# uci-rendering/psdr-cuda

Hardware: AMD Instinct MI355X
Metric: Mpath-samples/s renderC+renderD, cbox 512x512 spp=64; grad rel-L2 vs ref (higher is better)
Workload: dtype f32; 1 GPU; cbox 512x512 spp=64/GPU PathTracer(max_depth=3): renderC + configure + renderD + enoki.forward w.r.t. diffuse albedo, through the psdr_cuda surface; triangles=12, global_spp=64, world_size=1, device=AMD Radeon Graphics, local_rank=0

## Files before the change

__graft_entry__.py:

```python
import os
import subprocess
import sys

ROOT = os.path.dirname(os.path.abspath(__file__))
PKG = os.path.join(ROOT, "psdr-cuda_amd")
for p in (PKG, os.path.join(ROOT, "oracle"), os.path.join(ROOT, "tests")):
    if p not in sys.path:
        sys.path.insert(0, p)

HIPCC_FLAGS = ["--offload-arch=gfx950", "-O3", "-std=c++17", "-fPIC", "-munsafe-fp-atomics",
               "-fno-hip-fp32-correctly-rounded-divide-sqrt", "-fgpu-flush-denormals-to-zero", "-fno-slp-vectorize",
               "-freciprocal-math", "-fapprox-func"]
VARIANTS = (0, 1, 2, 3, 4, 6, 8, 10)


def _stale(target, sources):
    return (not os.path.exists(target)) or any(os.path.getmtime(s) > os.path.getmtime(target) for s in sources)


TESTS = os.path.join(ROOT, "tests")
CSRC = os.path.join(PKG, "csrc")
HC_DIR = os.path.join(TESTS, "hostcheck")
HOST_FLAGS = ["-O2", "-std=c++17", "-pthread"]


def _product_and_harness():
    return ([os.path.join(CSRC, f) for f in sorted(os.listdir(CSRC))] + [os.path.join(ROOT, "include", "psdr_hip.h")] +
            [os.path.join(HC_DIR, f) for f in sorted(os.listdir(HC_DIR)) if f.endswith(".h")])


TEST_LIBS = {
    "hostcheck": ("hostcheck/hostcheck.cpp", "hostcheck/libhostcheck.so", _product_and_harness, HOST_FLAGS),
    "path_sedge": ("hostcheck/hostcheck_path_sedge.cpp", "hostcheck/libhostcheck_path_sedge.so", _product_and_harness, HOST_FLAGS),
    "path_guide": ("hostcheck/hostcheck_path_guide.cpp", "hostcheck/libhostcheck_path_guide.so", _product_and_harness, HOST_FLAGS),
    "collocated": ("hostcheck/hostcheck_collocated.cpp", "hostcheck/libhostcheck_collocated.so", _product_and_harness, HOST_FLAGS),
    "pointlight": ("hostcheck/hostcheck_pointlight.cpp", "hostcheck/libhostcheck_pointlight.so", _product_and_harness, HOST_FLAGS),
    "lightstage": ("hostcheck/hostcheck_lightstage.cpp", "hostcheck/libhostcheck_lightstage.so", _product_and_harness, HOST_FLAGS),
    "distantlight": ("hostcheck/hostcheck_distantlight.cpp", "hostcheck/libhostcheck_distantlight.so", _product_and_harness, HOST_FLAGS),
    "plan": ("hostcheck/hostcheck_plan.cpp", "hostcheck/libhostcheck_plan.so", _product_and_harness, HOST_FLAGS),
    "smooth": ("hostcheck/hostcheck_smooth.cpp", "hostcheck/libhostcheck_smooth.so", lambda: [os.path.join(CSRC, "psdr_smooth.h")], HOST_FLAGS),
    "poison": ("poison/poison.hip", "poison/libpoison.so", lambda: [], ["-O1"]),
}


def testlib_deps(name):
    return [os.path.join(TESTS, TEST_LIBS[name][0])] + TEST_LIBS[name][2]()


def build_testlib(name):
    so = os.path.join(TESTS, TEST_LIBS[name][1])
    if _stale(so, testlib_deps(name)):
        subprocess.check_call(["hipcc", "--offload-arch=gfx950", "-fPIC", "-shared"] + TEST_LIBS[name][3] + [os.path.join(TESTS, TEST_LIBS[name][0]), "-o", so])
    return so


def build():
    csrc = os.path.join(PKG, "csrc")
    srcs = [os.path.join(csrc, f) for f in os.listdir(csrc)] + [os.path.join(ROOT, "include", "psdr_hip.h")]
    lib = os.path.join(PKG, "lib", "libpsdr_hip.so")
    os.makedirs(os.path.dirname(lib), exist_ok=True)
    defect_job = None
    if _stale(lib, srcs):
        obj_dir = os.path.join(PKG, "lib", "obj")
        os.makedirs(obj_dir, exist_ok=True)
        jobs, objs, unit_cmds = [], [], {}
        for v in VARIANTS:
            o = os.path.join(obj_dir, "variant%d.o" % v)
            objs.append(o)
            unit_cmds[o] = ["hipcc"] + HIPCC_FLAGS + ["-DPSDR_VARIANT_FLAGS=%d" % v, "-c", os.path.join(csrc, "psdr_variant.hip"), "-o", o]
            jobs.append(subprocess.Popen(unit_cmds[o]))
            o = os.path.join(obj_dir, "path_sedge%d.o" % v)
            objs.append(o)
            unit_cmds[o] = ["hipcc"] + HIPCC_FLAGS + ["-DPSDR_VARIANT_FLAGS=%d" % v, "-c", os.path.join(csrc, "psdr_path_sedge.hip"), "-o", o]
            jobs.append(subprocess.Popen(unit_cmds[o]))
            o = os.path.join(obj_dir, "collocated%d.o" % v)
            objs.append(o)
            unit_cmds[o] = ["hipcc"] + HIPCC_FLAGS + ["-DPSDR_VARIANT_FLAGS=%d" % v, "-c", os.path.join(csrc, "psdr_collocated.hip"), "-o", o]
            jobs.append(subprocess.Popen(unit_cmds[o]))
            o = os.path.join(obj_dir, "pointlight%d.o" % v)
            objs.append(o)
            unit_cmds[o] = ["hipcc"] + HIPCC_FLAGS + ["-DPSDR_VARIANT_FLAGS=%d" % v, "-c", os.path.join(csrc, "psdr_pointlight.hip"), "-o", o]
            jobs.append(subprocess.Popen(unit_cmds[o]))
            o = os.path.join(obj_dir, "lightstage%d.o" % v)
            objs.append(o)
            unit_cmds[o] = ["hipcc"] + HIPCC_FLAGS + ["-DPSDR_VARIANT_FLAGS=%d" % v, "-c", os.path.join(csrc, "psdr_lightstage.hip"), "-o", o]
            jobs.append(subprocess.Popen(unit_cmds[o]))
        o = os.path.join(obj_dir, "logd_lean.o")
        objs.append(o)
        unit_cmds[o] = ["hipcc"] + HIPCC_FLAGS + ["-c", os.path.join(csrc, "psdr_logd_lean.hip"), "-o", o]
        jobs.append(subprocess.Popen(unit_cmds[o]))
        o = os.path.join(obj_dir, "host.o")
        objs.append(o)
        unit_cmds[o] = ["hipcc"] + HIPCC_FLAGS + ["-c", os.path.join(csrc, "psdr_hip.hip"), "-o", o]
        jobs.append(subprocess.Popen(unit_cmds[o]))
        o = os.path.join(obj_dir, "tables.o")
        objs.append(o)
        unit_cmds[o] = ["hipcc"] + HIPCC_FLAGS + ["-c", os.path.join(csrc, "psdr_tables.hip"), "-o", o]
        jobs.append(subprocess.Popen(unit_cmds[o]))
        o = os.path.join(obj_dir, "smooth.o")
        objs.append(o)
        unit_cmds[o] = ["hipcc"] + HIPCC_FLAGS + ["-c", os.path.join(csrc, "psdr_smooth.hip"), "-o", o]
        jobs.append(subprocess.Popen(unit_cmds[o]))
        defect_job = _start_defect_object(csrc, obj_dir)
        if any(j.wait() != 0 for j in jobs):
            raise RuntimeError("hipcc failed")
        sys.path.insert(0, os.path.join(ROOT, "tools"))
        import check_spill_exec
        fallbacks = (["-mllvm", "-amdgpu-opt-exec-mask-pre-ra=0"], ["-mllvm", "-amdgpu-spill-sgpr-to-vgpr=0"])
        from concurrent.futures import ThreadPoolExecutor
        with ThreadPoolExecutor(max_workers=8) as pool:
            first = dict(zip(unit_cmds, pool.map(lambda o_: check_spill_exec.check_library(o_, verbose=True, min_code_objects=1), list(unit_cmds))))
        for o, cmd in list(unit_cmds.items()):
            hits = first[o]
            for extra in fallbacks:
                if not hits:
                    break
                print("build(): %s trips the spill guard -- rebuilding it with %s" % (os.path.basename(o), " ".join(extra)))
                subprocess.check_call(cmd[:1] + cmd[1:-4] + extra + cmd[-4:])
                hits = check_spill_exec.check_library(o, verbose=True, min_code_objects=1)
            if hits:
                raise RuntimeError("%s: %d kernel(s) spill in front of an exec restore with every fallback (tools/check_spill_exec.py)" % (os.path.basename(o), len(hits)))
        subprocess.check_call(["hipcc", "--offload-arch=gfx950", "-shared", "-fPIC"] + objs + ["-o", lib])
        if len(check_spill_exec.code_objects(lib)) < len(objs):
            raise RuntimeError("the linked library holds fewer gfx code objects than translation units: the spill guard cannot see all of it")
    subprocess.check_call(["make", "-C", os.path.join(ROOT, "oracle"), "-s"])
    for name in TEST_LIBS:
        build_testlib(name)
    try:
        build_defect_lib(defect_job)
    except Exception as e:
        print("build(): tests/poison/libpsdr_hip_defect.so not built (%s) -- only tests/test_rough_rev_order_gpu.py uses it" % e)
    import psdr_cuda
    from psdr_cuda import _abi
    _abi.load_hip()
    import oracle
    oracle.load_oracle()


def _defect_object_cmd(csrc, obj_dir):
    return ["hipcc"] + HIPCC_FLAGS + ["-DPSDR_VARIANT_FLAGS=10", "-DPSDR_SINK_REG_PRIV_ROUGH=1", "-DPSDR_DPP_ALWAYS=1", "-c",
                                      os.path.join(csrc, "psdr_variant.hip"), "-o", os.path.join(obj_dir, "variant10_defect.o")]


def _start_defect_object(csrc, obj_dir):
    try:
        return subprocess.Popen(_defect_object_cmd(csrc, obj_dir), stdout=subprocess.DEVNULL, stderr=subprocess.DEVNULL)
    except Exception:
        return None


def build_defect_lib(object_job=None):
    csrc = os.path.join(PKG, "csrc")
    srcs = [os.path.join(csrc, f) for f in os.listdir(csrc)] + [os.path.join(ROOT, "include", "psdr_hip.h")]
    obj_dir = os.path.join(PKG, "lib", "obj")
    defect_lib = os.path.join(ROOT, "tests", "poison", "libpsdr_hip_defect.so")
    objs = [os.path.join(obj_dir, "%s%d.o" % (unit, v)) for v in VARIANTS for unit in ("variant", "path_sedge", "collocated", "pointlight", "lightstage")] + [os.path.join(obj_dir, "logd_lean.o"), os.path.join(obj_dir, "host.o"), os.path.join(obj_dir, "tables.o"), os.path.join(obj_dir, "smooth.o")]
    if not all(os.path.exists(o) for o in objs):
        return None
    if object_job is not None and object_job.wait() != 0:
        object_job = None
    if _stale(defect_lib, srcs + objs):
        defect_obj = os.path.join(obj_dir, "variant10_defect.o")
        if object_job is None:
            subprocess.check_call(_defect_object_cmd(csrc, obj_dir))
        subprocess.check_call(["hipcc", "--offload-arch=gfx950", "-shared", "-fPIC"] + [defect_obj if o.endswith("variant10.o") else o for o in objs] + ["-o", defect_lib])
    return defect_lib


def smoke():
    import numpy as np
    import torch
    assert torch.cuda.is_available(), "smoke() needs a GPU"
    torch.cuda.set_device(0)
    import oracle
    from helpers import GpuScene, load_scene, rel_l2, tangents_wrt
    from psdr_cuda import _abi
    sc, P = load_scene("cbox", res=32, spp=8, sppe=4, sppse=4, translate=(0, (1.0, 0.0, 0.0)))
    tb = sc.tables(0)
    g = GpuScene(tb)
    o = _abi.make_opts(integrator=_abi.INTEGRATOR_PATH, max_depth=3, spp=8)
    img = g.render_c(o)
    ref = oracle.render(tb, o)
    assert np.isfinite(img).all() and rel_l2(img, ref) < 1e-4, rel_l2(img, ref)
    o = _abi.make_opts(spp=8, sppe=4, sppse=4)
    tan = tangents_wrt(tb, P)
    img, dimg = g.render_d_fwd(o, [tan])
    rimg, rd = oracle.render(tb, o, mode=1, tangents=tan)
    assert rel_l2(img, rimg) < 1e-4 and rel_l2(dimg[0], rd) < 1e-3, (rel_l2(img, rimg), rel_l2(dimg[0], rd))
    import psdr_cuda
    from psdr_cuda.fixtures import scene_path
    s2 = psdr_cuda.Scene()
    s2.load_file(scene_path("cbox"), False)
    s2.opts.width = s2.opts.height = 32
    s2.opts.spp, s2.opts.sppe, s2.opts.sppse, s2.opts.log_level = 4, 0, 0, 0
    s2.configure()
    out = psdr_cuda.DirectIntegrator(1, 1).renderC(s2).numpy()
    assert out.shape == (32 * 32, 3) and np.isfinite(out).all() and out.mean() > 0.05
    print("smoke OK: renderC rel-L2 vs oracle %.2e" % rel_l2(img, rimg))


if __name__ == "__main__":
    build()
    if len(sys.argv) > 1 and sys.argv[1] == "smoke":
        smoke()
    if len(sys.argv) > 1 and sys.argv[1] == "defect":
        print(build_defect_lib())
```

include/psdr_hip.h:

```cpp
#ifndef PSDR_HIP_H
#define PSDR_HIP_H

#include <stdint.h>

#ifdef __cplusplus
extern "C" {
#endif

#define PSDR_TRI_STRIDE   24
#define PSDR_TRIUV_STRIDE  8
#define PSDR_SEDGE_STRIDE 16
#define PSDR_PEDGE_STRIDE  8
#define PSDR_BSDF_STRIDE  16
#define PSDR_EMITTER_F_STRIDE 8
#define PSDR_EMITTER_I_STRIDE 4
#define PSDR_CAM_WORDS    64
#define PSDR_ENV_WORDS    32

#define PSDR_TRI_FACE_NORMALS 0x40000000

#define PSDR_BSDF_DIFFUSE        0
#define PSDR_BSDF_ROUGHCONDUCTOR 1
#define PSDR_BSDF_MICROFACET     2
#define PSDR_BSDF_MICROFACET_NORMAL 3
// ... 70 lines not shown
    const int32_t *sec_edge_faces;
    const float   *prim_edge_z;
} psdr_scene_desc;

#define PSDR_FLAG_FUSED     1
#define PSDR_FLAG_WAVEFRONT 2
#define PSDR_FLAG_LITERAL_FORMS 4
#define PSDR_FLAG_KEEP_RECORDS 8
#define PSDR_FLAG_PATH_SEDGES 16
#define PSDR_PATH_SEDGES_MAX_DEPTH 8

typedef struct psdr_render_opts {
    int32_t integrator;
    int32_t bsdf_samples, light_samples;
    int32_t max_depth;
    int32_t hide_emitters;
    int32_t field;
    int32_t spp, sppe, sppse;
    int32_t spp_begin, spp_end;
    int32_t sppe_begin, sppe_end;
    int32_t sppse_begin, sppse_end;
    int32_t flags;
    uint64_t rng_offset[3];
} psdr_render_opts;

typedef struct psdr_tangents {
    const float *d_tri_info;
    const float *d_texels;
    const float *d_emitter_rad;
    const float *d_cam_to_world;
    const float *d_sec_edge;
    const float *d_prim_edge;
    const float *d_env_f;
} psdr_tangents;

typedef struct psdr_grads {
    float *g_tri_info;
    float *g_texels;
    float *g_emitter_rad;
    float *g_cam_to_world;
    float *g_sec_edge;
    float *g_prim_edge;
    float *g_env_f;
} psdr_grads;

typedef struct psdr_scene_s *psdr_scene_t;

const char *psdr_last_error(void);
const char *psdr_version(void);
int psdr_abi_struct_sizes(int32_t out[4]);

int psdr_scene_create(psdr_scene_t *out);
int psdr_scene_destroy(psdr_scene_t h);
int psdr_scene_set_option(psdr_scene_t h, const char *name, double value);

int psdr_scene_set_tables(psdr_scene_t h, const psdr_scene_desc *desc);

int psdr_bvh_build(psdr_scene_t h, void *stream);
int psdr_bvh_stats(psdr_scene_t h, int32_t out[4]);
int psdr_scene_info(psdr_scene_t h, int32_t out[8]);

int psdr_trace(psdr_scene_t h, int32_t m,
               const float *ox, const float *oy, const float *oz,
               const float *dx, const float *dy, const float *dz,
               const float *tmax,
               int32_t *out_shape, int32_t *out_tri, float *out_u, float *out_v,
               void *stream);

int psdr_render_c(psdr_scene_t h, const psdr_render_opts *opts,
                  float *out_img, void *stream);

int psdr_render_d_fwd(psdr_scene_t h, const psdr_render_opts *opts,
                      int32_t K, const psdr_tangents *tangents,
                      float *out_img, float *out_dimg, void *stream);

int psdr_render_d_rev(psdr_scene_t h, const psdr_render_opts *opts,
                      const float *adj_img, float *out_img,
                      const psdr_grads *grads, void *stream);

int psdr_guide_build(psdr_scene_t h, const psdr_render_opts *opts,
                     const int32_t reso[4], int32_t nrounds,
                     float *out_mass, void *stream);

int psdr_scene_set_path_guide(psdr_scene_t h, const int32_t reso[3], const float *cmf, const float *pmf, float sum);
int psdr_scene_set_point_light(psdr_scene_t h, const float pos[3], int32_t K, const float *d_pos, float *g_pos);
int psdr_scene_set_point_lights(psdr_scene_t h, int32_t L, const float *pos, int32_t K, const float *d_pos, float *g_pos);
int psdr_scene_set_light(psdr_scene_t h, int32_t kind, const float v[3], int32_t K, const float *d_v, float *g_v);
int psdr_scene_set_lights(psdr_scene_t h, int32_t L, const int32_t *kinds, const float *v, int32_t K, const float *d_v, float *g_v);
int psdr_path_guide_build(psdr_scene_t h, const psdr_render_opts *opts, int32_t segment,
                          const int32_t reso[4], int32_t nrounds,
                          float *out_mass, void *stream);

int psdr_cube_sample_reuse(int32_t ndim, const int32_t *reso, const float *cmf, const float *pmf, float sum,
                           int32_t n, int32_t m, float *samples, float *out_pdf, void *stream);
int psdr_sample_boundary_segment_direct(const psdr_scene_desc *desc, int32_t m, const float *sample3,
                                        const uint8_t *active, float *out_p0, float *out_edge_dir,
                                        float *out_edge2, float *out_p2, float *out_n, float *out_pdf,
                                        uint8_t *out_valid, int32_t *out_edge, float *out_s1, void *stream);

int psdr_geo_world_vertices_fwd(int32_t V, const float *v_raw, const int32_t *vmesh, const float *mats, float *v_world, void *stream);
int psdr_geo_world_vertices_rev(int32_t V, const float *v_raw, const int32_t *vmesh, const float *mats, const float *v_world, const float *a_world, float *a_raw,
                                void *stream);
int psdr_geo_world_vertices_jvp(int32_t V, const float *v_raw, const int32_t *vmesh, const float *mats, const float *v_world, const float *t_raw, const float *t_mats,
                                float *t_world, void *stream);
int psdr_geo_tri_rows_fwd(int32_t V, int32_t T, const float *v, const int32_t *faces, float *vsum, float *rows, int32_t row_stride, void *stream);
int psdr_geo_tri_rows_rev(int32_t V, int32_t T, const float *v, const int32_t *faces, const float *vsum, const float *a_rows, int32_t row_stride,
                          float *a_vsum , float *a_v, void *stream);
int psdr_geo_tri_rows_jvp(int32_t V, int32_t T, const float *v, const int32_t *faces, const float *vsum, const float *t_v, int32_t row_stride,
                          float *t_vsum , float *t_rows, void *stream);
int psdr_geo_sec_edges_fwd(int32_t E, const int32_t *edges, const float *v, const float *rows, int32_t row_stride, float *info, uint8_t *keep, void *stream);
int psdr_geo_sec_edges_rev(int32_t E, const int32_t *edges, const float *a_info, float *a_v, float *a_rows, int32_t row_stride, void *stream);
int psdr_geo_sec_edges_jvp(int32_t E, const int32_t *edges, const float *t_v, const float *t_rows, int32_t row_stride, float *t_info, void *stream);
int psdr_geo_prim_edges_fwd(int32_t E, const int32_t *edges, const uint8_t *face_normals, const float *v, const float *rows, int32_t row_stride,
                            const float *cam22, float *rows8, float *z4, uint8_t *keep, void *stream);
int psdr_geo_prim_edges_rev(int32_t E, const int32_t *edges, const float *v, const float *cam22, const float *a_rows8, float *a_v, float *a_w2s ,
                            void *stream);
int psdr_geo_prim_edges_jvp(int32_t E, const int32_t *edges, const float *v, const float *cam22, const float *t_v, const float *t_w2s , float *t_rows8,
                            void *stream);

int psdr_geo_compact_edges_fwd(int32_t E, const float *rows, int32_t S, const uint8_t *keep, int32_t w0, int32_t wn, const void *aux, int32_t aux_stride, int32_t A,
                               void *scratch, float *rows_out, void *aux_out, int32_t *pos, float *pmf, float *cmf, float *header, void *stream);
int psdr_geo_compact_edges_rev(int32_t E, int32_t S, const int32_t *pos, const float *a_rows_out, float *a_rows, void *stream);
int psdr_geo_compact_edges_jvp(int32_t E, int32_t S, const int32_t *pos, const float *t_rows, float *t_rows_out, void *stream);
int psdr_geo_emitter_tables(int32_t M, const float *rows, int32_t row_stride, const int32_t *face_offset, const int32_t *mesh_emitter, int32_t Ne, const int32_t *emitter_i,
                            const float *radiance, const float *env_weight, float *mesh_area, float *emitter_f, float *emitter_pmf, float *emitter_cmf, float *face_pmf,
                            float *face_cmf, void *stream);

typedef struct psdr_smooth_s *psdr_smooth_t;
typedef struct psdr_smooth_info_s {
    int32_t iterations;
    int32_t converged;
    int32_t form;
    int32_t launches;
    float rel_residual[3];
    int32_t one_workgroup_limit;
    int32_t one_workgroup_default;
    int32_t num_vertices;
    int32_t num_entries;
    int32_t long_rows;
} psdr_smooth_info_t;
int psdr_smooth_create(int32_t V, int32_t F, const int32_t *faces, psdr_smooth_t *out);
void psdr_smooth_destroy(psdr_smooth_t h);
int psdr_smooth_set_option(psdr_smooth_t h, const char *name, int value);
int psdr_smooth_apply(psdr_smooth_t h, float lambda, const float *x, float *u, void *stream);
int psdr_smooth_solve(psdr_smooth_t h, float lambda, const float *b, const float *x0, float *x, float tol, int32_t max_iter, void *stream);
int psdr_smooth_info(psdr_smooth_t h, psdr_smooth_info_t *out);

int psdr_scene_rev_layout(psdr_scene_t h, int32_t out[16]);

int psdr_scene_seed_info(psdr_scene_t h, int64_t out[4]);

int psdr_scene_logd_info(psdr_scene_t h, int64_t out[4]);

int psdr_get_counters(psdr_scene_t h, uint64_t out[4]);

#ifdef __cplusplus
}
#endif
#endif
```

psdr-cuda_amd/csrc/psdr_hip.hip:

```cpp
#define PSDR_WIDE_TREE 2
#include "psdr_host.h"
#include "psdr_bvh_build.h"

#include <cstdlib>
#include <cstring>
#include <rocprim/rocprim.hpp>

namespace {
__global__ __launch_bounds__(kBlock) void k_trace(LaunchCtx cx, int m, const float *__restrict__ ox, const float *__restrict__ oy,
                                                  const float *__restrict__ oz, const float *__restrict__ dx,
                                                  const float *__restrict__ dy, const float *__restrict__ dz,
                                                  const float *__restrict__ tmax, int32_t *__restrict__ out_shape,
                                                  int32_t *__restrict__ out_tri, float *__restrict__ out_u, float *__restrict__ out_v) {
    TraversalStack st; setup_lds(cx, st);
    const SceneView &sc = cx.sc;
    for (int i = blockIdx.x * kBlock + threadIdx.x; i < m; i += gridDim.x * kBlock) {
        const Hit h = closest_hit<false, -1>(sc, st, Vec3f{ox[i], oy[i], oz[i]}, Vec3f{dx[i], dy[i], dz[i]}, tmax[i]);
        out_tri[i] = h.tri;
        out_shape[i] = h.tri >= 0 ? (sc.d.tri_mesh[h.tri] & ~PSDR_TRI_FACE_NORMALS) : -1;
        out_u[i] = h.u; out_v[i] = h.v;
    }
}


// ... 589 lines not shown
        HIP_TRY(hipMemcpyAsync(host_nodes.data(), h->d_nodes, host_nodes.size() * sizeof(BvhNode), hipMemcpyDeviceToHost, s));
        HIP_TRY(hipStreamSynchronize(s));
        if (int rc = bvh4_build(h, host_nodes, std::vector<int32_t>{0}, false, s)) return rc;
    } else { h->wide = false; h->num_nodes4 = 0; h->stack_need4 = 0; }
    h->level_start.clear();
    finish_build(h, T, info.pad, area, true, true);
    return 0;
}

int bvh4_refill(psdr_scene_s *h, hipStream_t s) {
    if (h->num_nodes4 <= 0) return 0;
    hipLaunchKernelGGL(k_bvh4_fill, dim3((h->num_nodes4 + kBlock - 1) / kBlock), dim3(kBlock), 0, s, h->d_nodes4, h->d_nodes, h->d_topo4,
                       h->d_topo4 + (size_t) h->num_nodes4 * 4, h->num_nodes4);
    HIP_TRY(hipGetLastError());
    return 0;
}
int bvh4_build(psdr_scene_s *h, const std::vector<BvhNode> &nodes, const std::vector<int32_t> &roots2, bool forest, hipStream_t s) {
    h->wide = use_wide_tree(h, forest);
    if (!h->wide && !forest) { h->num_nodes4 = 0; h->stack_need4 = 0; return 0; }
    Bvh4Topology tp;
    collapse_bvh4(nodes, roots2, tp);
    h->num_nodes4 = tp.n4; h->stack_need4 = tp.stack_need;
    h->root4 = roots2.size() == 1 ? tp.roots[0] : 0;
    for (size_t k = 0; k < roots2.size() && k < (size_t) kMaxBlas; ++k) h->blas_root4[k] = tp.roots[k];
    if (tp.n4 == 0) return 0;
    if (int rc = device_grow(h->d_nodes4, h->cap_nodes4, (size_t) tp.n4, sizeof(Bvh4Node), &h->d_topo4, 8 * sizeof(int32_t))) return rc;
    HIP_TRY(hipMemcpyAsync(h->d_topo4, tp.child.data(), (size_t) tp.n4 * 4 * sizeof(int32_t), hipMemcpyHostToDevice, s));
    HIP_TRY(hipMemcpyAsync(h->d_topo4 + (size_t) tp.n4 * 4, tp.src.data(), (size_t) tp.n4 * 4 * sizeof(int32_t), hipMemcpyHostToDevice, s));
    if (int rc = bvh4_refill(h, s)) return rc;
    HIP_TRY(hipStreamSynchronize(s));
    return 0;
}

int launch_wf_trace(psdr_scene_s *h, const float4 *req, const int32_t *count, long long sub_cap, float4 *hit, hipStream_t s, bool ign) {
    TraceArgs a{};
    a.sec_edge_faces = h->desc.sec_edge_faces;
    if (ign && !a.sec_edge_faces) ign = false;
    pack_blas_boxes(h, a.blas_lo, a.blas_hi);
    a.nodes4 = h->d_nodes4; a.btris = h->d_btris; a.req = req; a.count = count; a.hit = hit; a.sub_cap = sub_cap; a.n_blas = h->n_blas;
    const TracePlan p = plan_wf_trace(h, sub_cap);
    a.n_lnodes = p.n_lnodes; a.off_stack = p.off_stack; a.stack_entries = p.stack_entries; a.ovf_stride = p.ovf_stride;
    if (p.ovf) {
        if (int rc = scratch_reserve(reinterpret_cast<void **>(&h->d_trace_ovf), &h->trace_ovf_bytes, p.ovf_bytes, s, "trace kernel's overflow stack columns")) return rc;
        a.ovf = h->d_trace_ovf;
    }
    const bool wg2 = p.wg2, ovf = p.ovf;
    const int grid = p.grid, dyn = p.dyn;
#define PSDR_LAUNCH_TRACE_I(MULTI, OVF, IGN, WPE)                                                                                                           \
    do { static bool attr_set = false;                                                                                                                      \
         if (!attr_set) { if (int rc = allow_dynamic_lds(&k_wf_trace<MULTI, OVF, IGN, WPE>, 160 * 1024 - 1024)) return rc; attr_set = true; }                     \
         hipLaunchKernelGGL(HIP_KERNEL_NAME(k_wf_trace<MULTI, OVF, IGN, WPE>), dim3(grid), dim3(kTraceBlock), dyn, s, a); } while (0)
#define PSDR_LAUNCH_TRACE(MULTI, OVF) do { if (ign) { if (wg2) PSDR_LAUNCH_TRACE_I(MULTI, OVF, true, 8); else PSDR_LAUNCH_TRACE_I(MULTI, OVF, true, 4); } else if (wg2) PSDR_LAUNCH_TRACE_I(MULTI, OVF, false, 8); else PSDR_LAUNCH_TRACE_I(MULTI, OVF, false, 4); } while (0)
    if (h->n_blas > 1) { if (ovf) PSDR_LAUNCH_TRACE(true, true); else PSDR_LAUNCH_TRACE(true, false); }
    else { if (ovf) PSDR_LAUNCH_TRACE(false, true); else PSDR_LAUNCH_TRACE(false, false); }
#undef PSDR_LAUNCH_TRACE_I
#undef PSDR_LAUNCH_TRACE
    HIP_TRY(hipGetLastError());
    return 0;
}

int probe_buffers(psdr_scene_s *h, long long slots, int rays_per_slot, ProbeBuffers &pb, hipStream_t s, int per_cu) {
    const ProbePlan pl = plan_probe_buffers(h, slots, rays_per_slot, per_cu);
    pb.sub_cap = pl.sub_cap;
    if (int rc = scratch_reserve(&h->d_probe, &h->probe_bytes, pl.total, s, "probe buffers (hit rows, masks, trace requests)")) return rc;
    char *p = reinterpret_cast<char *>(h->d_probe);
    pb.count = reinterpret_cast<int32_t *>(p); p += pl.cnt_bytes;
    pb.hit = reinterpret_cast<float4 *>(p); p += pl.hit_bytes;
    pb.mask = reinterpret_cast<uint32_t *>(p); p += pl.mask_bytes;
    pb.req = reinterpret_cast<float4 *>(p);
    HIP_TRY(hipMemsetAsync(pb.count, 0, pl.cnt_bytes, s));
    return 0;
}

#define PSDR_OPS_OF(OPS)                                                                                                              \
    switch (scene_flag_set(h)) {                                                                                                      \
        case 0: return OPS##0(); case 1: return OPS##1(); case 2: return OPS##2(); case 3: return OPS##3();                          \
        case 4: return OPS##4(); case 8: return OPS##8(); case 10: return OPS##10();                                                 \
        default: return OPS##6();                       \
    }
const VariantOps *variant_of(const psdr_scene_s *h) { PSDR_OPS_OF(variant_ops_) }
const PathSedgeOps *path_sedge_of(const psdr_scene_s *h) { PSDR_OPS_OF(path_sedge_ops_) }
const CollocatedOps *collocated_of(const psdr_scene_s *h) { PSDR_OPS_OF(collocated_ops_) }
const PointLightOps *point_light_of(const psdr_scene_s *h) { PSDR_OPS_OF(point_light_ops_) }
const LightStageOps *light_stage_of(const psdr_scene_s *h) { PSDR_OPS_OF(light_stage_ops_) }
const char *const kDistantInEnv = "a distant light cannot reach a scene inside an environment map's bounding mesh (env_emitter >= 0)";
int check_point_light(const psdr_scene_s *h, const psdr_render_opts *o) {
    if (o->integrator == PSDR_INTEGRATOR_POINT && !h->have_point) return fail("PointLightIntegrator: no light set (psdr_scene_set_point_light)");
    if (o->integrator == PSDR_INTEGRATOR_POINT_STACK && h->stack_pos.empty()) return fail("LightStageIntegrator: no lights set (psdr_scene_set_point_lights)");
    if (h->desc.env_emitter >= 0) {
        const bool distant = o->integrator == PSDR_INTEGRATOR_POINT ? h->point_kind == PSDR_LIGHT_DISTANT
                           : o->integrator == PSDR_INTEGRATOR_POINT_STACK && std::find(h->stack_kind.begin(), h->stack_kind.end(), PSDR_LIGHT_DISTANT) != h->stack_kind.end();
        if (distant) return fail(kDistantInEnv);
    }
    return 0;
}
#undef PSDR_OPS_OF
}
using namespace psdr_host;

extern "C" {

const char *psdr_last_error(void) { return g_err.c_str(); }
const char *psdr_version(void) { return "psdr-hip 0.1 gfx950"; }
int psdr_abi_struct_sizes(int32_t out[4]) {
    out[0] = (int32_t) sizeof(psdr_scene_desc); out[1] = (int32_t) sizeof(psdr_render_opts);
    out[2] = (int32_t) sizeof(psdr_tangents); out[3] = (int32_t) sizeof(psdr_grads);
    return 0;
}

int psdr_scene_create(psdr_scene_t *out) {
    if (!out) return fail("psdr_scene_create: null output");
    psdr_scene_s *h = new psdr_scene_s();
    hipError_t e = hipMalloc(&h->d_counters, sizeof(unsigned long long) * kRayCounters * kRayCounterStride);
    if (e != hipSuccess) { delete h; return fail(std::string("hipMalloc: ") + hipGetErrorString(e)); }
    int dev = 0; hipDeviceProp_t prop;
    if (hipGetDevice(&dev) == hipSuccess && hipGetDeviceProperties(&prop, dev) == hipSuccess) {
        h->num_cus = prop.multiProcessorCount;
        h->lds_limit = (int) std::min<size_t>(prop.sharedMemPerBlock, 160 * 1024);
    }
    *out = h;
    return 0;
}

int psdr_scene_set_option(psdr_scene_t h, const char *name, double value) {
    if (!h || !name) return fail("psdr_scene_set_option: null argument");
    const std::string n(name);
    const int iv = (int) value;
    if (n == "bvh_refit") h->refit_enabled = iv != 0;
    else if (n == "forest_min_inline") { h->forest_min_inline = iv; h->have_bvh = false; }
    else if (n == "scratch_plain") g_scratch_plain = iv;
    else if (n == "own_pixels") h->opt.own_pixels = iv;
    else if (n == "emitter_pretest") h->opt.emitter_pretest = iv;
    else if (n == "occ_rows") { h->opt.occ_rows = iv; h->have_bvh = false; }
    else if (n == "aa_prims") { h->aa_enabled = iv != 0; h->have_bvh = false; }
    else if (n == "tiny_scene") h->tiny_enabled = iv != 0;
    else if (n == "two_level") h->two_level_enabled = iv != 0;
    else if (n == "wf_binned") h->wf_binned = iv != 0;
    else if (n == "wf_traced") h->traced_enabled = iv != 0;
    else if (n == "bvh_build") h->bvh_device_mode = iv;
    else if (n == "sort_edges") h->sort_edges = iv != 0;
    else if (n == "blocks_per_cu") h->opt.blocks_per_cu = iv;
    else if (n == "camera_blocks") h->opt.camera_blocks = iv;
    else if (n == "tiny_variants") h->opt.tiny_variants = iv;
    else if (n == "wide") h->opt.wide = iv;
    else if (n == "lds_budget") h->opt.lds_budget = iv;
    else if (n == "sink_rep") h->opt.sink_rep = std::max(1, std::min(16, iv));
    else if (n == "sink_private") h->opt.sink_private = iv;
    else if (n == "rev_split") h->opt.rev_split = iv;
    else if (n == "tangent_live") h->opt.tangent_live = iv;
    else if (n == "wf_geo") h->opt.wf_geo = iv;
    else if (n == "logd") h->opt.logd = iv;
    else if (n == "seed_cache") h->opt.seed_cache = iv;
    else if (n == "logd_park") h->opt.logd_park = iv;
    else if (n == "seed_cache_log2") h->opt.seed_cache_log2 = std::max(0, std::min(40, iv));
    else if (n == "keep_records") h->opt.keep_records = iv;
    else if (n == "rev_sorted") h->opt.rev_sorted = iv;
    else if (n == "sedge_split") h->opt.sedge_split = iv;
    else if (n == "pt_sedge") h->opt.pt_sedge = iv & 3;
    else if (n == "pt_sedge_walk") h->opt.pt_sedge_walk = iv;
    else if (n == "probe") h->opt.probe = iv;
    else if (n == "trace_wg2") h->opt.trace_wg2 = iv;
    else if (n == "chunk_log2") h->opt.chunk_log2 = std::max(0, std::min(30, iv));
    else if (n == "bvh_maxleaf") h->opt.bvh_maxleaf = std::max(1, std::min(8, iv));
    else if (n == "bvh_tcost") h->opt.bvh_tcost = (float) value;
    else return fail("psdr_scene_set_option: unknown option '" + n + "'");
    h->kept.valid = false;
    if (n == "tiny_scene" || n == "two_level" || n == "bvh_build" || n == "wide" || n == "bvh_maxleaf" || n == "bvh_tcost" || n == "tiny_variants") h->have_bvh = false;
    return 0;
}

int psdr_scene_destroy(psdr_scene_t h) {
    if (!h) return 0;
    if (h->d_nodes) (void) hipFree(h->d_nodes);
    if (h->d_stack_lights) (void) hipFree(h->d_stack_lights);
    if (h->d_btris) (void) hipFree(h->d_btris);
    if (h->d_counters) (void) hipFree(h->d_counters);
    if (h->d_refit_area) (void) hipFree(h->d_refit_area);
    if (h->d_sort) (void) hipFree(h->d_sort);
    if (h->d_ws) (void) hipFree(h->d_ws);
    if (h->d_live) (void) hipFree(h->d_live);
    if (h->d_logd_bad) (void) hipFree(h->d_logd_bad);
    if (h->d_seed) (void) hipFree(h->d_seed);
    if (h->seed_event) (void) hipEventDestroy(h->seed_event);
    if (h->d_hot_map) (void) hipFree(h->d_hot_map);
    if (h->d_hot_tris) (void) hipFree(h->d_hot_tris);
    if (h->d_occ) (void) hipFree(h->d_occ);
    if (h->d_top) (void) hipFree(h->d_top);
    if (h->d_inline_ids) (void) hipFree(h->d_inline_ids);
    if (h->d_lbvh) (void) hipFree(h->d_lbvh);
    if (h->d_nodes4) (void) hipFree(h->d_nodes4);
    if (h->d_topo4) (void) hipFree(h->d_topo4);
    if (h->d_rev) (void) hipFree(h->d_rev);
    if (h->d_se_list) (void) hipFree(h->d_se_list);
    if (h->d_rev_deep) (void) hipFree(h->d_rev_deep);
    if (h->d_pe_rep) (void) hipFree(h->d_pe_rep);
    if (h->d_trace_ovf) (void) hipFree(h->d_trace_ovf);
    if (h->d_probe) (void) hipFree(h->d_probe);
    delete h;
    return 0;
}

int psdr_scene_set_tables(psdr_scene_t h, const psdr_scene_desc *desc) {
    if (!h || !desc) return fail("psdr_scene_set_tables: null argument");
    psdr_scene_desc d = *desc;
    if (d.num_tris <= 0 || !d.tri_info || !d.tri_mesh) return fail("Missing meshes!");
    if (!d.cam) return fail("Missing sensor!");
    if (reinterpret_cast<uintptr_t>(d.tri_info) & 15) return fail("psdr_scene_set_tables: tri_info must be 16-byte aligned");
    if (d.width <= 0 || d.height <= 0) return fail("Invalid film resolution");
    if (d.num_meshes <= 0 || !d.mesh_bsdf || !d.mesh_emitter) return fail("psdr_scene_set_tables: mesh_bsdf / mesh_emitter missing");
    if (d.num_bsdfs > 0 && (!d.bsdf_rec || !d.texels)) return fail("psdr_scene_set_tables: bsdf_rec / texels missing");
    if (d.num_emitters > 0 && (!d.emitter_f || !d.emitter_i)) return fail("psdr_scene_set_tables: emitter tables missing");
    if (d.num_emitters > 1 && (!d.emitter_cmf || !d.emitter_pmf)) return fail("psdr_scene_set_tables: emitter distribution missing");
    if (d.num_sec_edges > 0 && (!d.sec_edge || !d.sec_cmf || !d.sec_pmf)) return fail("psdr_scene_set_tables: secondary-edge tables missing");
    if (d.num_prim_edges > 0 && (!d.prim_edge || !d.prim_cmf || !d.prim_pmf)) return fail("psdr_scene_set_tables: primary-edge tables missing");
    if (d.num_prim_edges <= 0) d.prim_edge_z = nullptr;
    if (d.num_guide_cells > 0 && (!d.guide_cmf || !d.guide_pmf)) return fail("psdr_scene_set_tables: guiding tables missing");
    if (!d.env_f) d.env_emitter = -1;
    if (d.env_emitter >= 0) {
        if (d.env_emitter >= d.num_emitters || !d.env_cmf || !d.env_pmf || d.env_reso[0] <= 0 || d.env_reso[1] <= 0 || d.env_tex[1] < 2 ||
            d.env_tex[2] < 2)
            return fail("psdr_scene_set_tables: inconsistent environment-map record");
    }
    if (h->have_tables && (d.tri_info != h->desc.tri_info || d.num_tris != h->desc.num_tris)) h->have_bvh = false;
    if (h->have_tables && (d.emitter_i != h->desc.emitter_i || d.num_emitters != h->desc.num_emitters)) h->have_bvh = false;
    if (!h->have_tables || std::memcmp(&h->desc, &d, sizeof(d)) != 0) { ++h->tables_gen; h->kept.valid = false; }
    h->desc = d;
    h->has_microfacet = (d.material_mask & ((1u << PSDR_BSDF_MICROFACET) | (1u << PSDR_BSDF_MICROFACET_NORMAL) | (1u << PSDR_BSDF_MICROFACET_HEIGHT))) != 0;
    h->has_rough = d.material_mask == 0 || (d.material_mask & (1u << PSDR_BSDF_ROUGHCONDUCTOR)) != 0 || h->has_microfacet;
    h->have_tables = true;
    h->pg_cmf = h->pg_pmf = nullptr; h->pg_sum = 0.f;
    return 0;
}

int psdr_scene_set_path_guide(psdr_scene_t h, const int32_t reso[3], const float *cmf, const float *pmf, float sum) {
    if (!h) return fail("psdr_scene_set_path_guide: null argument");
    if (!cmf) { h->pg_cmf = h->pg_pmf = nullptr; h->pg_sum = 0.f; return 0; }
    if (!reso || !pmf) return fail("psdr_scene_set_path_guide: null argument");
    if (reso[0] <= 0 || reso[1] <= 0 || reso[2] <= 0 || (long long) reso[0] * reso[1] * reso[2] > 0x7fffffffLL) return fail("psdr_scene_set_path_guide: invalid resolution");
    for (int i = 0; i < 3; ++i) h->pg_reso[i] = reso[i];
    h->pg_cmf = cmf; h->pg_pmf = pmf; h->pg_sum = sum;
    return 0;
}

static hipError_t copy_on_stream(void *dst, const void *src, size_t bytes, hipMemcpyKind kind, hipStream_t s) {
    if (hipError_t e = hipMemcpyAsync(dst, src, bytes, kind, s)) return e;
    return hipStreamSynchronize(s);
}
static void update_emit_rows(psdr_scene_s *h) {
    h->emit_rows = 0;
    if (h->n_tiny > 0 && emit_rows_wanted(h))
        h->emit_rows = tiny_emitter_rows(h->tiny_meta, h->n_tiny, h->aa_cnt, emitter_triangle_mask(h->emitter_i, h->desc.num_emitters, h->desc.num_tris));
}

static void refit_done(psdr_scene_s *h) { h->refits_since_build++; h->num_refits++; h->have_bvh = true; }
static int emitters_unchanged(psdr_scene_s *h, hipStream_t s, bool &same) {
    same = (size_t) std::max(h->desc.num_emitters, 0) * PSDR_EMITTER_I_STRIDE == h->emitter_i.size();
    if (!same || h->emitter_i.empty()) return 0;
    same = h->desc.emitter_i != nullptr;
    if (!same) return 0;
    std::vector<int32_t> now(h->emitter_i.size());
    HIP_TRY(copy_on_stream(now.data(), h->desc.emitter_i, now.size() * sizeof(int32_t), hipMemcpyDeviceToHost, s));
    same = std::memcmp(now.data(), h->emitter_i.data(), now.size() * sizeof(int32_t)) == 0;
    return 0;
}
static int host_tree_refit(psdr_scene_s *h, hipStream_t s, bool &fits) {
    fits = true;
    HIP_TRY(hipMemsetAsync(h->d_refit_area, 0, sizeof(float), s));
    hipLaunchKernelGGL(k_refit_leaves, dim3((h->num_btris + kBlock - 1) / kBlock), dim3(kBlock), 0, s, h->d_btris, h->desc.tri_info, h->num_btris);
    for (int l = (int) h->level_start.size() - 2; l >= 0; --l) {
        const int first = h->level_start[l], count = h->level_start[l + 1] - first;
        hipLaunchKernelGGL(k_refit_level, dim3((count + kBlock - 1) / kBlock), dim3(kBlock), 0, s, h->d_nodes, h->d_btris, first, count, h->bvh_pad, h->d_refit_area);
    }
    HIP_TRY(hipGetLastError());
    if (int rc = bvh4_refill(h, s)) return rc;
    if (h->n_blas == 0) return 0;
    float4 top[kMaxInlineTris * 3 + 2 * kMaxBlas];
    hipLaunchKernelGGL(k_gather_top, dim3(1), dim3(64), 0, s, h->d_top, h->d_nodes, h->desc.tri_info, h->d_inline_ids, h->n_inline, h->n_blas);
    HIP_TRY(hipMemcpyAsync(top, h->d_top, sizeof(top), hipMemcpyDeviceToHost, s));
    HIP_TRY(hipStreamSynchronize(s));
    std::vector<float4> tris(top, top + 3 * (size_t) h->n_inline), prims;
    pack_tiny_prims(tris, prims);
    fits = refit_inline_fits((int) prims.size() / 3);
    if (!fits) return 0;
    h->n_tiny = tiny_plane_form(prims, h->tiny, h->tiny_meta, &h->aa_cnt, h->aa_enabled);
    update_emit_rows(h);
    for (int k = 0; k < h->n_blas; ++k) {
        const float w = h->blas_lo[k].w;
        h->blas_lo[k] = top[kMaxInlineTris * 3 + k]; h->blas_lo[k].w = w;
        h->blas_hi[k] = top[kMaxInlineTris * 3 + kMaxBlas + k];
    }
    return 0;
}
static int try_refit(psdr_scene_s *h, int T, bool tiny, hipStream_t s, bool &done) {
    done = false;
    if (!refit_candidate(h, T, tiny)) return 0;
    bool emitters_same = false;
    if (int rc = emitters_unchanged(h, s, emitters_same)) return rc;
    const bool stands = forest_stands(h);
    if (refit_choice(h, emitters_same, stands, h->built_area) == kRefitNone) return 0;
    float prev_area = h->built_area;
    if (h->refits_since_build > 0) {
        HIP_TRY(hipMemcpyAsync(&prev_area, h->d_refit_area, sizeof(float), hipMemcpyDeviceToHost, h->refit_stream));
        HIP_TRY(hipStreamSynchronize(h->refit_stream));
    }
    const RefitKind kind = refit_choice(h, emitters_same, stands, prev_area);
    if (kind == kRefitNone) return 0;
// ... 228 lines not shown
    if (pos == nullptr || L == 0) return 0;
    if (int rc = device_grow(h->d_stack_lights, h->cap_stack_lights, (size_t) L, sizeof(float) * 13)) return rc;
    h->stack_pos.assign(pos, pos + 3 * (size_t) L);
    h->stack_kind.assign((size_t) L, PSDR_LIGHT_POINT);
    if (d_pos != nullptr && K > 0) { h->stack_K = K; h->stack_dpos.assign(d_pos, d_pos + 3 * (size_t) L * K); }
    h->stack_gpos = g_pos;
    return 0;
}

static int check_light_vector(const char *fn, int kind, const float *v, const std::string &which) {
    if (kind != PSDR_LIGHT_POINT && kind != PSDR_LIGHT_DISTANT) return fail(std::string(fn) + ": unknown light kind " + std::to_string(kind) + which + " (PSDR_LIGHT_POINT or PSDR_LIGHT_DISTANT)");
    if (kind != PSDR_LIGHT_DISTANT || v == nullptr) return 0;
    if (!(std::isfinite(v[0]) && std::isfinite(v[1]) && std::isfinite(v[2]))) return fail(std::string(fn) + ": the direction" + which + " is not finite");
    if (v[0] == 0.f && v[1] == 0.f && v[2] == 0.f) return fail(std::string(fn) + ": the direction" + which + " is all zero");
    return 0;
}

int psdr_scene_set_light(psdr_scene_t h, int32_t kind, const float v[3], int32_t K, const float *d_v, float *g_v) {
    if (!h) return fail("psdr_scene_set_light: null handle");
    if (int rc = check_light_vector("psdr_scene_set_light", kind, v, "")) return rc;
    if (int rc = psdr_scene_set_point_light(h, v, K, d_v, g_v)) return rc;
    if (v != nullptr) h->point_kind = kind;
    return 0;
}

int psdr_scene_set_lights(psdr_scene_t h, int32_t L, const int32_t *kinds, const float *v, int32_t K, const float *d_v, float *g_v) {
    if (!h) return fail("psdr_scene_set_lights: null handle");
    const bool some = v != nullptr && L != 0;
    if (some && kinds == nullptr) return fail("psdr_scene_set_lights: null kinds");
    if (some && L >= 1 && L <= PSDR_POINT_LIGHTS_MAX)
        for (int l = 0; l < L; ++l)
            if (int rc = check_light_vector("psdr_scene_set_lights", kinds[l], v + 3 * l, " of light " + std::to_string(l))) return rc;
    if (int rc = psdr_scene_set_point_lights(h, L, v, K, d_v, g_v)) return rc;
    if (some) h->stack_kind.assign(kinds, kinds + L);
    return 0;
}

int psdr_guide_build(psdr_scene_t h, const psdr_render_opts *o, const int32_t reso[4], int32_t nrounds, float *out_mass, void *stream) {
    if (!h || !o || !reso || !out_mass) return fail("psdr_guide_build: null argument");
    if (int rc = check_microfacet(h, o)) return rc;
    if (nrounds <= 0) return fail("psdr_guide_build: nrounds must be positive");
    if (h->desc.num_sec_edges <= 0) return fail("psdr_guide_build: scene has no secondary edges");
    hipStream_t s = (hipStream_t) stream;
    if (int rc = begin_call(h, s)) return rc;
    LaunchCtx cx;
    if (int rc = make_ctx(h, o, 2, cx)) return rc;
    cx.sc.d.guide_cmf = nullptr; cx.sc.d.num_guide_cells = 0;
    const long long cells = (long long) reso[0] * reso[1] * reso[2];
    const long long n = cells * reso[3];
    if (n <= 0 || n > 0x7fffffffLL) return fail("psdr_guide_build: invalid resolution");
    HIP_TRY(hipMemsetAsync(out_mass, 0, sizeof(float) * cells, s));
    return variant_of(h)->guide(h, cx, reso, nrounds, n, out_mass, s);
}

int psdr_path_guide_build(psdr_scene_t h, const psdr_render_opts *o, int32_t segment, const int32_t reso[4], int32_t nrounds, float *out_mass, void *stream) {
    if (!h || !o || !reso || !out_mass) return fail("psdr_path_guide_build: null argument");
    if (int rc = check_microfacet(h, o)) return rc;
    if (nrounds <= 0) return fail("psdr_path_guide_build: nrounds must be positive");
    if (o->integrator != PSDR_INTEGRATOR_PATH) return fail("psdr_path_guide_build: the integrator must be PSDR_INTEGRATOR_PATH");
    if (o->max_depth < 1) return fail("psdr_path_guide_build: max_depth must be at least 1");
    if (o->max_depth > PSDR_PATH_SEDGES_MAX_DEPTH) return fail("psdr_path_guide_build: PathTracer max_depth > 8 is not supported for the secondary-edge term");
    if (segment != 1 && segment != 2) return fail("psdr_path_guide_build: segment must be 1 (direct source) or 2 (indirect source)");
    if (segment == 2 && o->max_depth < 2) return fail("psdr_path_guide_build: segment 2 needs max_depth >= 2");
    if (!h->have_tables) return fail("Scene not loaded yet!");
    if (h->desc.num_sec_edges <= 0) return fail("psdr_path_guide_build: scene has no secondary edges");
    if (reso[0] <= 0 || reso[1] <= 0 || reso[2] <= 0 || reso[3] <= 0) return fail("psdr_path_guide_build: invalid resolution");
    const long long cells = (long long) reso[0] * reso[1] * reso[2];
    if (cells > 0x7fffffffLL || cells * reso[3] > 0x7fffffffLL || cells * reso[3] * (long long) nrounds > 0x7fffffffLL)
        return fail("psdr_path_guide_build: more than 2^31 (stream, round) slots");
    hipStream_t s = (hipStream_t) stream;
    if (int rc = begin_call(h, s)) return rc;
    HIP_TRY(hipMemsetAsync(out_mass, 0, sizeof(float) * cells, s));
    return path_sedge_of(h)->guide(h, o, segment, reso, nrounds, out_mass, s);
}

int psdr_cube_sample_reuse(int32_t ndim, const int32_t *reso, const float *cmf, const float *pmf, float sum, int32_t n, int32_t m, float *samples,
                           float *out_pdf, void *stream) {
    if (!reso || !cmf || !pmf || !samples || !out_pdf) return fail("psdr_cube_sample_reuse: null argument");
    if (ndim != 2 && ndim != 3) return fail("psdr_cube_sample_reuse: ndim must be 2 or 3");
    long long cells = 1;
    for (int d = 0; d < ndim; ++d) {
        if (reso[d] <= 0) return fail("psdr_cube_sample_reuse: invalid resolution");
        cells *= reso[d];
    }
    if (cells != (long long) n) return fail("psdr_cube_sample_reuse: n must be the product of the resolution");
    if (m < 0) return fail("psdr_cube_sample_reuse: negative sample count");
    if (m == 0) return 0;
    const dim3 grid((unsigned) ((m + kBlock - 1) / kBlock));
    hipStream_t s = (hipStream_t) stream;
    if (ndim == 2)
        hipLaunchKernelGGL(k_cube_sample_reuse<2>, grid, dim3(kBlock), 0, s, m, cmf, pmf, sum, n, reso[0], reso[1], 1, samples, out_pdf);
    else
        hipLaunchKernelGGL(k_cube_sample_reuse<3>, grid, dim3(kBlock), 0, s, m, cmf, pmf, sum, n, reso[0], reso[1], reso[2], samples, out_pdf);
    HIP_TRY(hipGetLastError());
    return 0;
}

int psdr_sample_boundary_segment_direct(const psdr_scene_desc *desc, int32_t m, const float *sample3, const uint8_t *active, float *out_p0,
                                        float *out_edge_dir, float *out_edge2, float *out_p2, float *out_n, float *out_pdf, uint8_t *out_valid,
                                        int32_t *out_edge, float *out_s1, void *stream) {
    if (!desc || !sample3 || !out_p0 || !out_edge_dir || !out_edge2 || !out_p2 || !out_n || !out_pdf || !out_valid || !out_edge || !out_s1)
        return fail("psdr_sample_boundary_segment_direct: null argument");
    const psdr_scene_desc &d = *desc;
    if (d.num_sec_edges <= 0 || !d.sec_edge || !d.sec_cmf || !d.sec_pmf) return fail("Scene has no secondary edges");
    if (d.num_emitters <= 0 || !d.emitter_f || !d.emitter_i) return fail("No Emitter!");
    if (d.num_emitters > 1 && (!d.emitter_cmf || !d.emitter_pmf)) return fail("psdr_sample_boundary_segment_direct: emitter distribution missing");
    const bool env = d.env_f != nullptr && d.env_emitter >= 0;
    if (env && (d.env_emitter >= d.num_emitters || !d.env_cmf || !d.env_pmf || d.env_reso[0] <= 0 || d.env_reso[1] <= 0))
        return fail("psdr_sample_boundary_segment_direct: inconsistent environment-map record");
    if (d.num_emitters > (env ? 1 : 0) && (d.num_tris <= 0 || !d.tri_info || !d.face_cmf || !d.face_pmf))
        return fail("psdr_sample_boundary_segment_direct: area-light tables missing");
    if (m < 0) return fail("psdr_sample_boundary_segment_direct: negative sample count");
    if (m == 0) return 0;
    SceneView sc{};
    sc.d = d;
    if (!env) sc.d.env_emitter = -1;
    const dim3 grid((unsigned) ((m + kBlock - 1) / kBlock));
    hipStream_t s = (hipStream_t) stream;
    if (env)
        hipLaunchKernelGGL(k_boundary_segment_direct<kSceneEnv>, grid, dim3(kBlock), 0, s, sc, m, sample3, active, out_p0, out_edge_dir, out_edge2, out_p2, out_n,
                           out_pdf, out_valid, out_edge, out_s1);
    else
        hipLaunchKernelGGL(k_boundary_segment_direct<0>, grid, dim3(kBlock), 0, s, sc, m, sample3, active, out_p0, out_edge_dir, out_edge2, out_p2, out_n,
                           out_pdf, out_valid, out_edge, out_s1);
    HIP_TRY(hipGetLastError());
    return 0;
}

int psdr_bvh_stats(psdr_scene_t h, int32_t out[4]) {
    if (!h || !out) return fail("psdr_bvh_stats: null argument");
    out[0] = h->num_builds; out[1] = h->num_refits; out[2] = h->num_nodes; out[3] = h->bvh_depth;
    return 0;
}

int psdr_scene_info(psdr_scene_t h, int32_t out[8]) {
    if (!h || !out) return fail("psdr_scene_info: null argument");
    const int n_slab = (h->aa_cnt & 255) + ((h->aa_cnt >> 8) & 255) + (h->aa_cnt >> 16);
    out[0] = h->n_tiny - (h->aa_cnt != 0 ? kAaSlots - n_slab : 0); out[1] = h->n_blas; out[2] = h->n_inline; out[3] = h->num_btris; out[4] = h->lbvh ? 1 : 0;
    out[5] = n_slab; out[6] = h->have_occ ? 1 : 0; out[7] = h->have_occ ? h->occ_max_rows : 0;
    return 0;
}

int psdr_scene_rev_layout(psdr_scene_t h, int32_t out[16]) {
    if (!h || !out) return fail("psdr_scene_rev_layout: null argument");
    std::copy(std::begin(h->rev_layout), std::end(h->rev_layout), out);
    return 0;
}

int psdr_scene_logd_info(psdr_scene_t h, int64_t out[4]) {
    if (!h || !out) return fail("psdr_scene_logd_info: null argument");
    out[0] = h->logd_launches; out[1] = h->logd_lean_launches; out[2] = h->logd_lean_seeded; out[3] = (int64_t) h->logd_lean_lds + h->logd_lean_park;
    return 0;
}
int psdr_scene_seed_info(psdr_scene_t h, int64_t out[4]) {
    if (!h || !out) return fail("psdr_scene_seed_info: null argument");
    out[0] = h->seed_valid ? h->seed_key[0] * h->seed_key[3] : 0; out[1] = (int64_t) (h->seed_cap * sizeof(ulonglong2)); out[2] = h->seed_fills; out[3] = h->seed_launches;
    return 0;
}

int psdr_get_counters(psdr_scene_t h, uint64_t out[4]) {
    if (!h || !out) return fail("psdr_get_counters: null argument");
    unsigned long long all[kRayCounters * kRayCounterStride], c[1] = {0};
    HIP_TRY(hipMemcpyAsync(all, h->d_counters, sizeof(all), hipMemcpyDeviceToHost, h->last_stream));
    HIP_TRY(hipStreamSynchronize(h->last_stream));
    for (int i = 0; i < kRayCounters; ++i) c[0] += all[i * kRayCounterStride];
#ifdef PSDR_STAGE_CLOCKS
    {
        unsigned long long ph[12] = {0};
        for (int i = 0; i < kRayCounters; ++i) for (int k = 0; k < 12; ++k) ph[k] += all[i * kRayCounterStride + 1 + k];
        std::fprintf(stderr, "stage clocks:");
        for (int k = 0; k < 12; ++k) std::fprintf(stderr, " %llu", ph[k]);
        std::fprintf(stderr, "\n");
    }
#endif
    out[0] = c[0]; out[1] = h->slots[0]; out[2] = h->slots[1]; out[3] = h->slots[2];
    return 0;
}

}
```

psdr-cuda_amd/csrc/psdr_host.h:

```cpp
#pragma once
#include "psdr_device.h"
#include "psdr_reverse.h"

#include <algorithm>
#include <type_traits>
#include <cmath>
#include <cstdio>
#include <cstdlib>
#include <cstring>
#include <string>
#include <vector>

using namespace psdr;

struct LaunchCtx {
    SceneView sc;
    LiParams lp;
    RngJump jump;
    int32_t off_stack;
    int32_t off_pathrec;
    int32_t off_sink;
    int32_t off_park;
};

static_assert(offsetof(LaunchCtx, sc) == 0, "closest_hit reads SceneView::tiny through the kernel-argument segment pointer: LaunchCtx (SceneView first) must be the first kernel argument");

__device__ __forceinline__ void setup_lds(const LaunchCtx &cx, TraversalStack &st) {
#if defined(__HIP_DEVICE_COMPILE__)
    const SceneView &sc = cx.sc;
    float4 *dst = reinterpret_cast<float4 *>(psdr_dyn_lds);
    const float4 *src = sc.nodes4 != nullptr ? reinterpret_cast<const float4 *>(sc.nodes4) : reinterpret_cast<const float4 *>(sc.nodes);
    for (int i = threadIdx.x; i < sc.n_lnodes * 4; i += kBlock) dst[sc.off_lnodes / 16 + (i >> 2) * (kLdsNodeStride / 16) + (i & 3)] = src[i];
    for (int i = threadIdx.x; i < sc.n_lbtris * 3; i += kBlock) dst[sc.off_lbtris / 16 + i] = sc.btris[i];
    src = reinterpret_cast<const float4 *>(sc.d.tri_info);
    for (int i = threadIdx.x; i < sc.n_ltri * 6; i += kBlock) dst[sc.off_ltri / 16 + i] = src[i];
    {
        float *m = reinterpret_cast<float *>(psdr_dyn_lds + sc.off_lprim);
#pragma unroll 1
        for (int i = 0; i < sc.n_tiny; ++i) {
            int32_t tri; float k[6];
            const int w = threadIdx.x & 7;
            const float4 Sm = sc.tiny[i * 4 + 2];
            const float S[4] = {Sm.x, Sm.y, Sm.z, Sm.w};
            tiny_hit_row(sc.tiny_meta + i * 4, (threadIdx.x >> 3) & 1, tri, k, (sc.aa_cnt != 0 && i < kAaSlots) ? S : nullptr);
            const float val = w == 0 ? __int_as_float(tri) : (w == 1 ? k[0] : w == 2 ? k[1] : w == 3 ? k[2] : w == 4 ? k[3] : w == 5 ? k[4] : w == 6 ? k[5] : 0.f);
            if (threadIdx.x < kTinyHitWords) m[i * kTinyHitWords + threadIdx.x] = val;
        }
    }
    if (sc.lt_meshbsdf >= 0) {
        auto stage = [&](int off, const void *table, int words) {
            if (off < 0 || table == nullptr) return;
            const uint32_t *g = static_cast<const uint32_t *>(table);
            uint32_t *l = reinterpret_cast<uint32_t *>(psdr_dyn_lds + off);
#pragma unroll 1
            for (int i = threadIdx.x; i < words; i += kBlock) l[i] = g[i];
        };
        stage(sc.lt_trimesh, sc.d.tri_mesh, sc.d.num_tris);
        stage(sc.lt_meshbsdf, sc.d.mesh_bsdf, sc.d.num_meshes);
        stage(sc.lt_meshemitter, sc.d.mesh_emitter, sc.d.num_meshes);
        stage(sc.lt_bsdf, sc.d.bsdf_rec, sc.d.num_bsdfs * PSDR_BSDF_STRIDE);
        stage(sc.lt_emf, sc.d.emitter_f, sc.d.num_emitters * PSDR_EMITTER_F_STRIDE);
        stage(sc.lt_emi, sc.d.emitter_i, sc.d.num_emitters * PSDR_EMITTER_I_STRIDE);
        stage(sc.lt_ecmf, sc.d.emitter_cmf, sc.d.num_emitters);
        stage(sc.lt_epmf, sc.d.emitter_pmf, sc.d.num_emitters);
        stage(sc.lt_fcmf, sc.d.face_cmf, sc.lt_nfaces);
        stage(sc.lt_fpmf, sc.d.face_pmf, sc.lt_nfaces);
        stage(sc.lt_uv, sc.d.tri_uv, sc.d.num_tris * PSDR_TRIUV_STRIDE);
        stage(sc.lt_tex, sc.d.texels, sc.d.num_texels);
        stage(sc.lt_occ, sc.occ, sc.d.num_tris * sc.d.num_tris);
    }
    st.base = reinterpret_cast<int32_t *>(psdr_dyn_lds + cx.off_stack) + threadIdx.x;
    __syncthreads();
#else
    (void) cx; (void) st;
#endif
}
template <class TVT> __device__ __forceinline__ void setup_lds(const LaunchCtx &cx, TraversalStack &st, const TVT &tv) {
    setup_lds(cx, st);
#if defined(__HIP_DEVICE_COMPILE__)
    if constexpr (Tab<TVT::flags>::lds_small && TVT::k > 0) {
        constexpr int K = TVT::k;
        static_assert(K <= 3, "plan_lds reserves three tangent texel pools");
        if (cx.sc.lt_tex >= 0) {
            float *l = reinterpret_cast<float *>(psdr_dyn_lds + cx.sc.lt_tex);
            const int nt = cx.sc.d.num_texels;
            for (int k = 0; k < K; ++k) {
                const float *g = tv.t[k].d_texels;
                for (int i = threadIdx.x; i < nt; i += kBlock) l[(k + 1) * nt + i] = g ? g[i] : 0.f;
            }
            __syncthreads();
        }
    }
#endif
}

constexpr int kSinkCacheWords = 6144;
struct SinkLayout {
    int tex_off, tex_n;
    int rad_off, rad_n;
    int cam_off;
    int env_off, env_n;
    int hot_off, hot_rows;
    const int32_t *hot_map, *hot_tris;
    int total;
    int rep, stride;
    int priv_off, priv_rows;
    int priv_tri[2], priv_slot[2], priv_emitter;
    int priv_regs;
    int pend_off, pend_rows;
};
constexpr int kPendWords = 10;
constexpr int kPrivRowWords = 13;
constexpr int kPrivWords = 2 * kPrivRowWords + 3;

struct psdr_scene_options {
    int blocks_per_cu = 0;
    int camera_blocks = 0;
    int tiny_variants = 1;
    int wide = -1;
    int lds_budget = 0;
    int sink_rep = 4;
    int sink_private = 1;
    int rev_split = -1;
    int tangent_live = 1;
    int wf_geo = 1;
    int own_pixels = 1;
    int emitter_pretest = 1;
    int occ_rows = 1;
    int logd = 1;
    int keep_records = 1;
    int rev_sorted = 1;
    int pt_sedge = 3;
    int pt_sedge_walk = 1;
    int sedge_split = -1;
    int chunk_log2 = 0;
    int probe = 1;
    int trace_wg2 = -1;
    int seed_cache = 1;
    int seed_cache_log2 = 25;
    int logd_park = 1;
    int bvh_maxleaf = 4;
    float bvh_tcost = 2.0f;
};

struct psdr_scene_s {
    psdr_scene_options opt;
    psdr_scene_desc desc{};
    bool have_tables = false;
    bool has_rough = true;
    int num_cus = 256;
    int lds_limit = 64 * 1024;

    BvhNode *d_nodes = nullptr;
    float4 *d_btris = nullptr;
    size_t cap_nodes = 0, cap_btris = 0;
    int32_t root = 0;
    bool have_bvh = false;
    int bvh_depth = 0, num_nodes = 0, num_btris = 0;
    Bvh4Node *d_nodes4 = nullptr;
    int32_t *d_topo4 = nullptr;
    size_t cap_nodes4 = 0;
    int num_nodes4 = 0, stack_need4 = 0;
    bool wide = false;
    int32_t *d_trace_ovf = nullptr;
    size_t trace_ovf_bytes = 0;
    bool traced_enabled = true;
    int32_t root4 = 0, blas_root4[kMaxBlas] = {};
    bool refit_enabled = true;
    int tree_tris = -1, refits_since_build = 0, num_builds = 0, num_refits = 0;
    std::vector<int> level_start;
    float bvh_pad = 0.f, built_area = 0.f;
    float *d_refit_area = nullptr;

    int bvh_device_mode = -1;
    bool lbvh = false;
    int lbvh_leaves = 0;
    void *d_lbvh = nullptr;
    size_t lbvh_bytes = 0;

    bool tiny_enabled = true, aa_enabled = true;
    int n_tiny = 0, aa_cnt = 0;
    float4 tiny[kTinyRows * 4] = {};
    int32_t tiny_meta[kTinyRows * 4] = {};
    bool two_level_enabled = true, refit_ok = true, wf_binned = true;
    int n_blas = 0, n_inline = 0;
    float4 blas_lo[kMaxBlas] = {}, blas_hi[kMaxBlas] = {};
    float4 *d_top = nullptr;
    int32_t *d_inline_ids = nullptr;

    unsigned long long *d_counters = nullptr;
    hipStream_t last_stream = nullptr;
    hipStream_t refit_stream = nullptr;
    uint64_t slots[3] = {0, 0, 0};
    int last_path_depth = 0;
    int32_t rev_layout[16] = {};

    std::vector<int32_t> emitter_i;
    int32_t *d_hot_map = nullptr, *d_hot_tris = nullptr;
    uint32_t *d_occ = nullptr; size_t occ_cap = 0; bool have_occ = false; int occ_max_rows = 0;
    int hot_rows = 0;
    bool hot_identity = false;
    size_t hot_cap = 0;

    bool sort_edges = true;
    void *d_sort = nullptr;
    size_t sort_bytes = 0;

    void *d_pe_rep = nullptr;
    size_t pe_rep_bytes = 0;

    void *d_rev_deep = nullptr;
    size_t rev_deep_bytes = 0;

    void *d_se_list = nullptr;
    size_t se_list_bytes = 0;

    void *d_rev = nullptr;
    size_t rev_bytes = 0;
    void *d_logd_bad = nullptr; size_t logd_bad_bytes = 0;
    struct KeptRecords { bool valid = false; psdr_render_opts o{}; uint64_t gen = 0; long long n = 0; int kind = 0; } kept;
    uint64_t tables_gen = 0;

    void *d_seed = nullptr;
    size_t seed_cap = 0;
    long long seed_key[4] = {0, 0, 0, 0};
    bool seed_valid = false;
    hipStream_t seed_stream = nullptr;
    hipEvent_t seed_event = nullptr;
    long long seed_fills = 0, seed_launches = 0;
    long long logd_launches = 0, logd_lean_launches = 0, logd_lean_seeded = 0;
    int logd_lean_lds = 0, logd_lean_park = 0;
    void *d_ws = nullptr;
    size_t ws_bytes = 0;
    void *d_live = nullptr;
    size_t live_bytes = 0;
    void *d_probe = nullptr;
    size_t probe_bytes = 0;
    uint32_t emit_rows = 0;
    int forest_min_inline = 0;
    int32_t pg_reso[3] = {1, 1, 1};
    const float *pg_cmf = nullptr, *pg_pmf = nullptr;
    float pg_sum = 0.f;
    bool has_microfacet = false;
    bool have_point = false;
    float point_pos[3] = {0.f, 0.f, 0.f}, point_dpos[3][3] = {};
    int point_K = 0;
    float *point_gpos = nullptr;
    int point_kind = PSDR_LIGHT_POINT;
    std::vector<float> stack_pos, stack_dpos;
    int stack_K = 0;
    float *stack_gpos = nullptr;
    std::vector<int32_t> stack_kind;
    float *d_stack_lights = nullptr;
    size_t cap_stack_lights = 0;
};

constexpr int kRayCounters = 64, kRayCounterStride = 16;
constexpr int kWfSub = 64, kWfCountStride = 32;
constexpr int kTraceBlock = 1024, kTraceNodeStride = 80, kTraceStackMax = 16;

#define HIP_TRY(expr)                                                                              \
    do { hipError_t e_ = (expr); if (e_ != hipSuccess) return psdr_host::fail(std::string(#expr) + ": " + hipGetErrorString(e_)); } while (0)
namespace psdr_host {
int fail(const std::string &m);
template <class Kernel> int allow_dynamic_lds(Kernel *kernel, int bytes) {
    if (bytes > 48 * 1024) HIP_TRY(hipFuncSetAttribute(reinterpret_cast<const void *>(kernel), hipFuncAttributeMaxDynamicSharedMemorySize, bytes));
    return 0;
}
int scratch_reserve(void **buf, size_t *have, size_t need, hipStream_t s, const char *what);
long long fit_chunk(long long chunk, size_t bytes_per_slot, size_t fixed_bytes, size_t have);
inline int workspace_reserve(psdr_scene_s *h, size_t need, hipStream_t s) { return scratch_reserve(&h->d_ws, &h->ws_bytes, need, s, "wavefront workspace (path-state streams + trace requests)"); }
void fill_top(const psdr_scene_s *h, SceneView &sc);
constexpr int kMaxInlineTris = 2 * kTinyTris;
int make_ctx(psdr_scene_s *h, const psdr_render_opts *o, int sampler, LaunchCtx &cx);
int launch_wf_trace(psdr_scene_s *h, const float4 *req, const int32_t *count, long long sub_cap, float4 *hit, hipStream_t s, bool ign = false);
struct ProbeBuffers { float4 *hit; uint32_t *mask; float4 *req; int32_t *count; long long sub_cap; };
int probe_buffers(psdr_scene_s *h, long long slots, int rays_per_slot, ProbeBuffers &pb, hipStream_t s, int per_cu = 16);
inline int sink_bytes_base(const SinkLayout &L) { return (L.priv_rows > 0 && !L.priv_regs) ? (L.priv_off + kPrivWords * kBlock) * 4 : (L.rep * L.stride * 4 + 15) / 16 * 16; }
inline int sink_bytes(const SinkLayout &L) { return L.pend_rows > 0 ? (L.pend_off + L.pend_rows * kPendWords * kBlock) * 4 : sink_bytes_base(L); }
inline void sink_reserve_pending(SinkLayout &L, int rows) { L.pend_rows = 0; L.pend_off = (sink_bytes_base(L) / 4 + 3) / 4 * 4; L.pend_rows = rows; }
int check_counts(const psdr_scene_s *h, const psdr_render_opts *o);
int check_microfacet(const psdr_scene_s *h, const psdr_render_opts *o);
int begin_call(psdr_scene_s *h, hipStream_t s);
int primary_edge_order(psdr_scene_s *h, const LaunchCtx &cx, long long i0, long long n, const uint32_t **order, hipStream_t s);
constexpr int kMaxRefits = 64;
constexpr float kRefitAreaGrowth = 1.3f;
constexpr int kLbvhAutoTris = 1 << 18;

struct VariantOps {
    int (*render_c)(psdr_scene_s *h, const psdr_render_opts *o, float *img, hipStream_t s);
    int (*render_fwd)(psdr_scene_s *h, const psdr_render_opts *o, int K, const psdr_tangents *tangents, float *img, float *dimg, hipStream_t s);
    int (*render_rev)(psdr_scene_s *h, const psdr_render_opts *o, const float *adj_img, float *out_img, const psdr_grads *grads, hipStream_t s);
    int (*guide)(psdr_scene_s *h, LaunchCtx &cx, const int32_t reso[4], int nrounds, long long n, float *out_mass, hipStream_t s);
};
struct PathSedgeOps {
    int (*fwd)(psdr_scene_s *h, const psdr_render_opts *o, int K, const psdr_tangents *tangents, float *dimg, hipStream_t s);
    int (*rev)(psdr_scene_s *h, const psdr_render_opts *o, const float *adj_img, const psdr_grads *grads, hipStream_t s);
    int (*guide)(psdr_scene_s *h, const psdr_render_opts *o, int segment, const int32_t reso[4], int nrounds, float *out_mass, hipStream_t s);
};
const PathSedgeOps *path_sedge_ops_0();
const PathSedgeOps *path_sedge_ops_1();
const PathSedgeOps *path_sedge_ops_2();
const PathSedgeOps *path_sedge_ops_3();
const PathSedgeOps *path_sedge_ops_4();
const PathSedgeOps *path_sedge_ops_6();
const PathSedgeOps *path_sedge_ops_8();
const PathSedgeOps *path_sedge_ops_10();
struct CollocatedOps {
    int (*render_c)(psdr_scene_s *h, const psdr_render_opts *o, float *img, hipStream_t s);
    int (*render_fwd)(psdr_scene_s *h, const psdr_render_opts *o, int K, const psdr_tangents *tangents, float *img, float *dimg, hipStream_t s);
    int (*render_rev)(psdr_scene_s *h, const psdr_render_opts *o, const float *adj_img, float *out_img, const psdr_grads *grads, hipStream_t s);
};
const CollocatedOps *collocated_ops_0();
const CollocatedOps *collocated_ops_1();
const CollocatedOps *collocated_ops_2();
const CollocatedOps *collocated_ops_3();
const CollocatedOps *collocated_ops_4();
const CollocatedOps *collocated_ops_6();
const CollocatedOps *collocated_ops_8();
const CollocatedOps *collocated_ops_10();
struct PointLightOps {
    int (*render_c)(psdr_scene_s *h, const psdr_render_opts *o, float *img, hipStream_t s);
    int (*render_fwd)(psdr_scene_s *h, const psdr_render_opts *o, int K, const psdr_tangents *tangents, float *img, float *dimg, hipStream_t s);
    int (*render_rev)(psdr_scene_s *h, const psdr_render_opts *o, const float *adj_img, float *out_img, const psdr_grads *grads, hipStream_t s);
    int (*edges_fwd)(psdr_scene_s *h, const psdr_render_opts *o, int K, const psdr_tangents *tangents, int kind, const float *pos, const float *d_pos, float *dimg, long long plane, hipStream_t s);
    int (*edges_rev)(psdr_scene_s *h, const psdr_render_opts *o, const float *adj_img, const psdr_grads *grads, int kind, const float *pos, float *g_pos, hipStream_t s);
};
const PointLightOps *point_light_ops_0();
const PointLightOps *point_light_ops_1();
const PointLightOps *point_light_ops_2();
const PointLightOps *point_light_ops_3();
const PointLightOps *point_light_ops_4();
const PointLightOps *point_light_ops_6();
const PointLightOps *point_light_ops_8();
const PointLightOps *point_light_ops_10();
struct LightStageOps {
    int (*render_c)(psdr_scene_s *h, const psdr_render_opts *o, float *img, hipStream_t s);
    int (*render_fwd)(psdr_scene_s *h, const psdr_render_opts *o, int K, const psdr_tangents *tangents, float *img, float *dimg, const PointLightOps *point, hipStream_t s);
    int (*render_rev)(psdr_scene_s *h, const psdr_render_opts *o, const float *adj_img, float *out_img, const psdr_grads *grads, const PointLightOps *point, hipStream_t s);
};
const LightStageOps *light_stage_ops_0();
const LightStageOps *light_stage_ops_1();
const LightStageOps *light_stage_ops_2();
const LightStageOps *light_stage_ops_3();
const LightStageOps *light_stage_ops_4();
const LightStageOps *light_stage_ops_6();
const LightStageOps *light_stage_ops_8();
const LightStageOps *light_stage_ops_10();
int logd_lean_launch_8(psdr_scene_s *h, const psdr_render_opts *o, const LaunchCtx &cx, const psdr::TangentView<1, psdr::kSceneTiny> &tv, float *img, float *dimg, hipStream_t s, bool *ran);
const VariantOps *variant_ops_0();
const VariantOps *variant_ops_1();
const VariantOps *variant_ops_2();
const VariantOps *variant_ops_3();
const VariantOps *variant_ops_4();
const VariantOps *variant_ops_6();
const VariantOps *variant_ops_8();
const VariantOps *variant_ops_10();
}

#include "psdr_plan.h"
#include "psdr_tree_plan.h"
```

psdr-cuda_amd/csrc/psdr_kernels.h:

```cpp
#pragma once
#include "psdr_host.h"

namespace {
using namespace psdr_host;

__device__ __forceinline__ float wave_shfl_down(float v, int off) { return __shfl_down(v, off, 64); }

template <int CTRL, int ROW_MASK> __device__ __forceinline__ float dpp_add(float v) {
    return v + __int_as_float(__builtin_amdgcn_update_dpp(0, __float_as_int(v), CTRL, ROW_MASK, 0xf, true));
}
__device__ __forceinline__ float wave_total(float v) {
    v = dpp_add<0x111, 0xf>(v); v = dpp_add<0x112, 0xf>(v); v = dpp_add<0x114, 0xf>(v); v = dpp_add<0x118, 0xf>(v);
    v = dpp_add<0x142, 0xa>(v); v = dpp_add<0x143, 0xc>(v);
    return __int_as_float(__builtin_amdgcn_readlane(__float_as_int(v), 63));
}
#ifndef PSDR_DPP_ALWAYS
#define PSDR_DPP_ALWAYS 0
#endif
template <int N, bool DPP = (N <= 6 || PSDR_DPP_ALWAYS)> __device__ __forceinline__ bool wave_segmented_sum(int key, float (&v)[N]) {
    const int lane = threadIdx.x & 63;
    if (DPP && __ballot(key != __builtin_amdgcn_readfirstlane(key)) == 0ull) {
#pragma unroll
        for (int i = 0; i < N; ++i) v[i] = wave_total(v[i]);
        return lane == 0;
// ... 1453 lines not shown
__global__ __launch_bounds__(kBlock) void k_secondary_edge_rev(LaunchCtx cx, DeviceSink<FL> sink, long long i0, long long n, float inv_sppse,
                                                               const float *__restrict__ adj_img, unsigned long long *counters,
                                                               const uint32_t *__restrict__ list, const int *__restrict__ list_n) {
    TraversalStack st; setup_lds(cx, st);
    sink.begin(dyn_lds_floats(cx.off_sink));
    uint32_t nrays = 0;
    const bool guided = cx.sc.d.guide_cmf != nullptr && cx.sc.d.num_guide_cells > 0;
    if (list != nullptr) n = *list_n;
    for (long long jj = (long long) blockIdx.x * kBlock + threadIdx.x; jj < n; jj += (long long) gridDim.x * kBlock) {
        const long long j = list != nullptr ? (long long) list[jj] : jj;
        Rng rng; rng.init((uint64_t) (i0 + j), cx.jump);
        float s3[3] = {rng.next(), rng.next(), rng.next()};
        const float pdf0 = guided ? guide_sample_reuse(cx.sc, s3) : 1.f;
        secondary_edge_reverse(sink, cx.sc, st, s3, (pdf0 > kEpsilon ? 1.f / pdf0 : 1.f) * inv_sppse, adj_img, nrays, list == nullptr);
    }
    sink.end();
    count_rays(counters, nrays);
}


template <int FL> int make_device_sink(const psdr_scene_s *h, const psdr_grads *grads, DeviceSink<FL> &sink) {
    sink.g = *grads; sink.L = make_sink_layout(h, grads);
    if ((FL & kSceneTiny) != 0 && PSDR_TINY_DIRECT_ROWS && grads->g_tri_info != nullptr && !(h->hot_identity && sink.L.hot_rows == h->desc.num_tris))
        return fail("psdr_render_d_rev: the gradient cache of a scene without a tree does not hold every triangle row");
    return 0;
}
inline bool tangents_move_geometry(const psdr_tangents *tangents, int K) {
    bool geo = false;
    for (int k = 0; k < K; ++k) geo = geo || tangents[k].d_tri_info || tangents[k].d_cam_to_world;
    return geo;
}
struct EdgeLaunch { LaunchCtx cx; long long i0, n; const uint32_t *order; };
inline int begin_edge_term(psdr_scene_s *h, const psdr_render_opts *o, int sampler, EdgeLaunch &e, hipStream_t s) {
    if (int rc = make_ctx(h, o, sampler, e.cx)) return rc;
    const long long WH = (long long) h->desc.width * h->desc.height;
    const int begin = sampler == 1 ? o->sppe_begin : o->sppse_begin, end = sampler == 1 ? o->sppe_end : o->sppse_end;
    e.i0 = WH * begin; e.n = WH * (end - begin);
    h->slots[sampler] += (uint64_t) e.n;
    e.order = nullptr;
    return sampler == 1 ? primary_edge_order(h, e.cx, e.i0, e.n, &e.order, s) : 0;
}
template <int FL> int begin_pe_replicas(psdr_scene_s *h, const psdr_grads *grads, const EdgeLaunch &e, PrimaryEdgeSink<FL> &pe_sink, hipStream_t s) {
    const long long pe_words = (long long) h->desc.num_prim_edges * PSDR_PEDGE_STRIDE;
    const int reps = primary_edge_replicas(pe_words, e.n);
    if (reps > 1) {
        const size_t need = (size_t) reps * pe_words * sizeof(float);
        if (int rc = scratch_reserve(&h->d_pe_rep, &h->pe_rep_bytes, need, s, "primary-edge gradient replicas")) return rc;
        HIP_TRY(hipMemsetAsync(h->d_pe_rep, 0, need, s));
    }
    pe_sink = PrimaryEdgeSink<FL>{reps > 1 ? reinterpret_cast<float *>(h->d_pe_rep) : grads->g_prim_edge, pe_words, reps};
    h->rev_layout[9] = reps; h->rev_layout[15] = e.order != nullptr ? 1 : 0;
    return 0;
}
template <int FL> int end_pe_replicas(psdr_scene_s *h, const psdr_grads *grads, const PrimaryEdgeSink<FL> &pe_sink, hipStream_t s) {
    if (pe_sink.reps > 1) {
        hipLaunchKernelGGL(k_sum_replicas, dim3((unsigned) ((pe_sink.rep_stride + kBlock - 1) / kBlock)), dim3(kBlock), 0, s, grads->g_prim_edge,
                           reinterpret_cast<const float *>(h->d_pe_rep), pe_sink.rep_stride, pe_sink.reps);
        HIP_TRY(hipGetLastError());
    }
    return 0;
}
template <int FL> int probe_and_trace(psdr_scene_s *h, const psdr_render_opts *o, const LaunchCtx &cx, long long c0, long long nc, ProbeBuffers &pb, hipStream_t s) {
    const int probe_per_cu = big_launch_per_cu(h, nc);
    if (int rc = probe_buffers(h, nc, 3, pb, s, probe_per_cu)) return rc;
    const TraceQueue tq{pb.req, pb.count, pb.sub_cap};
    const int blocks = (launch_blocks(h, nc, probe_per_cu) + kWfSub - 1) / kWfSub * kWfSub;
    hipLaunchKernelGGL(k_direct_probe<FL>, dim3(blocks), dim3(kBlock), lds_bytes(cx, h), s, cx, TangentView<0, FL>{}, o->spp, o->spp_begin, SlotDiv(o->spp_end - o->spp_begin), c0, nc, tq,
                       pb.hit, pb.mask, make_rng_jump(o->rng_offset[0] + 2));
    HIP_TRY(hipGetLastError());
    return launch_wf_trace(h, pb.req, pb.count, pb.sub_cap, pb.hit, s);
}
inline const ulonglong2 *seed_table(psdr_scene_s *h, const psdr_render_opts *o, long long WH, int nsp, long long n, hipStream_t s) {
    if (h->opt.seed_cache == 0 || n <= 0 || n > (1ll << std::max(0, std::min(40, h->opt.seed_cache_log2)))) return nullptr;
    const long long key[4] = {WH, (long long) o->spp, (long long) o->spp_begin, (long long) nsp};
    if (h->d_seed != nullptr && h->seed_valid && std::equal(key, key + 4, h->seed_key)) {
        if (s != h->seed_stream && h->seed_event != nullptr && hipStreamWaitEvent(s, h->seed_event, 0) != hipSuccess) { (void) hipGetLastError(); return nullptr; }
        return reinterpret_cast<const ulonglong2 *>(h->d_seed);
    }
    h->seed_valid = false;
    if ((size_t) n > h->seed_cap) {
        if (h->d_seed) { (void) hipFreeAsync(h->d_seed, s); h->d_seed = nullptr; h->seed_cap = 0; }
        void *nb = nullptr;
        if (hipMallocAsync(&nb, (size_t) n * sizeof(ulonglong2), s) != hipSuccess) { (void) hipGetLastError(); return nullptr; }
        h->d_seed = nb; h->seed_cap = (size_t) n;
    }
    if (h->seed_event == nullptr && hipEventCreateWithFlags(&h->seed_event, hipEventDisableTiming) != hipSuccess) { (void) hipGetLastError(); h->seed_event = nullptr; return nullptr; }
    hipLaunchKernelGGL(k_seed_fill, dim3((unsigned) ((n + kBlock - 1) / kBlock)), dim3(kBlock), 0, s, reinterpret_cast<ulonglong2 *>(h->d_seed), n, o->spp, o->spp_begin, SlotDiv(nsp));
    if (hipGetLastError() != hipSuccess || hipEventRecord(h->seed_event, s) != hipSuccess) { (void) hipGetLastError(); return nullptr; }
    std::copy(key, key + 4, h->seed_key);
    h->seed_valid = true; h->seed_stream = s; h->seed_fills++;
    return reinterpret_cast<const ulonglong2 *>(h->d_seed);
}
template <class G, class R, int FL> constexpr bool seeded_render_c() { return (FL & kSceneTiny) != 0 && (FL & kScenePre) == 0 && std::is_same<G, float>::value && std::is_same<R, float>::value; }
template <class G, class R, int FL>
int run_camera(psdr_scene_s *h, const psdr_render_opts *o, const TV<R, FL> &tv, float *img, float *dimg, hipStream_t s) {
    const long long WH = (long long) h->desc.width * h->desc.height;
    const int nsp = o->spp_end - o->spp_begin;
    if (o->spp <= 0 || nsp <= 0) return 0;
    LaunchCtx cx;
    if (int rc = make_ctx(h, o, 0, cx)) return rc;
    const long long n = WH * nsp;
    h->slots[0] += (uint64_t) n;
    if constexpr ((FL & kSceneForest) != 0) {
        if (o->integrator == PSDR_INTEGRATOR_DIRECT && probe_direct(h, o, n)) {
            TV<R, FL | kScenePre> tvp;
            for (int k = 0; k < (ad_traits<R>::K > 0 ? ad_traits<R>::K : 1); ++k) tvp.t[k] = tv.t[k];
            tvp.live = tv.live;
            LaunchCtx cxp = cx;
            plan_lds_no_walk(h, cxp);
            const long long chunk = std::min<long long>(n, launch_chunk(h, 25));
            const int own = wave_owns_pixels(h, nsp, chunk);
            for (long long c0 = 0; c0 < n; c0 += chunk) {
                const long long nc = std::min(chunk, n - c0);
                ProbeBuffers pb;
                if (int rc = probe_and_trace<FL>(h, o, cx, c0, nc, pb, s)) return rc;
                hipLaunchKernelGGL(HIP_KERNEL_NAME(k_camera<G, R, PSDR_INTEGRATOR_DIRECT, FL | kScenePre, false>), dim3(launch_blocks(h, nc, camera_blocks_per_cu(h, nc))), dim3(kBlock), cxp.off_stack, s,
                                   cxp, tvp, o->spp, o->spp_begin, SlotDiv(nsp), nc, 1.f / (float) o->spp, img, dimg, WH * 3, h->d_counters, c0, ProbeView{pb.hit, pb.mask}, own);
                HIP_TRY(hipGetLastError());
            }
            return 0;
        }
    }
    const int own = wave_owns_pixels(h, nsp, n);
    bool gated = false;
    if constexpr (logd_instance<G, R, PSDR_INTEGRATOR_PATH, FL>()) {
        constexpr int K = ad_traits<R>::K;
        bool texels_only = o->integrator == PSDR_INTEGRATOR_PATH && h->opt.logd != 0 && h->desc.num_texels > 0 && h->desc.texels != nullptr;
        for (int k = 0; k < K && texels_only; ++k) {
            const psdr_tangents &t = tv.t[k];
            texels_only = t.d_texels != nullptr && !t.d_tri_info && !t.d_emitter_rad && !t.d_cam_to_world && !t.d_sec_edge && !t.d_prim_edge && !t.d_env_f;
        }
        if (texels_only) {
            if (int rc = scratch_reserve(&h->d_logd_bad, &h->logd_bad_bytes, sizeof(int), s, "log-derivative gate")) return rc;
            int *bad = reinterpret_cast<int *>(h->d_logd_bad);
            HIP_TRY(hipMemsetAsync(bad, 0, sizeof(int), s));
            TangentView<K, 0> tvk;
            for (int k = 0; k < K; ++k) tvk.t[k] = tv.t[k];
            hipLaunchKernelGGL(k_logd_check<K>, dim3((unsigned) ((h->desc.num_texels + kBlock - 1) / kBlock)), dim3(kBlock), 0, s, h->desc.texels, tvk, h->desc.num_texels, h->d_counters, bad);
            hipLaunchKernelGGL(k_logd_gate, dim3(1), dim3(64), 0, s, h->d_counters, bad);
            bool lean = false;
            if constexpr (K == 1 && FL == kSceneTiny) { if (int rc = logd_lean_launch_8(h, o, cx, tv, img, dimg, s, &lean)) return rc; }
            if (!lean)
                hipLaunchKernelGGL(HIP_KERNEL_NAME(k_camera_logd<K, FL, ((FL & kSceneTiny) != 0)>), dim3(launch_blocks(h, n, camera_blocks_per_cu(h, n))), dim3(kBlock), lds_bytes(cx, h), s, cx, tv,
                                   o->spp, o->spp_begin, SlotDiv(nsp), n, 1.f / (float) o->spp, img, dimg, WH * 3, h->d_counters, own);
            HIP_TRY(hipGetLastError());
            h->logd_launches++;
            gated = true;
        }
    }
#define PSDR_LAUNCH_CAMERA_T(INTEG, NOTREE)                                                                                        \
    hipLaunchKernelGGL(HIP_KERNEL_NAME(k_camera<G, R, INTEG, FL, NOTREE>), dim3(launch_blocks(h, n, camera_blocks_per_cu(h, n))), dim3(kBlock), lds_bytes(cx, h), s, cx, tv, o->spp, \
                       o->spp_begin, nsp, n, 1.f / (float) o->spp, img, dimg, WH * 3, h->d_counters, 0ll, ProbeView{nullptr, nullptr}, own)
#define PSDR_LAUNCH_CAMERA(INTEG) PSDR_LAUNCH_CAMERA_T(INTEG, ((FL & kSceneTiny) != 0))
    if constexpr (seeded_render_c<G, R, FL>()) {
        if (o->integrator == PSDR_INTEGRATOR_PATH) {
            if (const ulonglong2 *seed = seed_table(h, o, WH, nsp, n, s)) {
                hipLaunchKernelGGL(HIP_KERNEL_NAME(k_camera_seeded<G, R, PSDR_INTEGRATOR_PATH, FL, true>), dim3(launch_blocks(h, n, camera_blocks_per_cu(h, n))), dim3(kBlock), lds_bytes(cx, h), s, cx, tv,
                                   o->spp, o->spp_begin, SlotDiv(nsp), n, 1.f / (float) o->spp, img, dimg, WH * 3, h->d_counters, own, seed);
                HIP_TRY(hipGetLastError());
                h->seed_launches++;
                return 0;
            }
        }
    }
    switch (o->integrator) {
        case PSDR_INTEGRATOR_DIRECT: PSDR_LAUNCH_CAMERA(PSDR_INTEGRATOR_DIRECT); break;
        case PSDR_INTEGRATOR_PATH: PSDR_LAUNCH_CAMERA(PSDR_INTEGRATOR_PATH); break;
        case PSDR_INTEGRATOR_FIELD: PSDR_LAUNCH_CAMERA(PSDR_INTEGRATOR_FIELD); break;
        default: return fail("Unknown integrator");
    }
#undef PSDR_LAUNCH_CAMERA
#undef PSDR_LAUNCH_CAMERA_T
    HIP_TRY(hipGetLastError());
    if (gated) HIP_TRY(hipMemsetAsync(h->d_counters + kLogdGateWord, 0, sizeof(unsigned long long), s));
    return 0;
}


constexpr int kWfMaxDepth = 256;
struct WfRecArgs { float *disk; long long stride, c0, nc; };
template <class M, int FL>
int run_camera_wavefront(psdr_scene_s *h, const psdr_render_opts *o, const TV<M, FL> &tv, float *img, float *dimg, hipStream_t s, const WfRecArgs *rec = nullptr) {
    constexpr int K = ad_traits<M>::K;
    const long long WH = (long long) h->desc.width * h->desc.height;
    const int nsp = o->spp_end - o->spp_begin;
    if (o->spp <= 0 || nsp <= 0) return 0;
    const long long n_all = WH * nsp;
    const long long n = rec ? rec->nc : n_all;
    bool traced = false;
    if constexpr ((FL & kSceneForest) != 0) traced = traced_wavefront(h);
    const bool binned = !traced && (FL & kSceneForest) != 0 && h->n_blas > 0 && h->wf_binned;
    const int depth = o->max_depth;
    const size_t words = 8 + 6 * (1 + K) + (traced ? 8 : 0);
    const long long cap = rec ? n : std::min(n, fit_chunk(binned ? launch_chunk(h, 24) : launch_chunk(h, traced ? 26 : 25), 2 * words * 4 * 5 / 4 + (traced ? 80 : 0), 64u << 20, h->ws_bytes));
    const auto wf_per_cu = [&](long long slots) { return traced ? big_launch_per_cu(h, slots) : 16; };
    const long long max_blocks = ((long long) launch_blocks(h, cap, wf_per_cu(cap)) + kWfSub - 1) / kWfSub * kWfSub;
    const long long binned_sub_cap = (((cap + kBlock - 1) / kBlock + kWfSub) / kWfGroups + 2) * kBlock;
    const long long cap_alloc = ((binned ? binned_sub_cap * kWfSub : cap + max_blocks * kBlock) + 63) / 64 * 64;
    const size_t cnt_ints = (size_t) (kWfMaxDepth + 1) * kWfStageInts + (traced ? (size_t) (kWfMaxDepth + 1) * kWfSub * kWfCountStride : 0);
    const size_t cnt_bytes = cnt_ints * sizeof(int32_t);
    const size_t req_bytes = traced ? (size_t) 2 * cap_alloc * 2 * sizeof(float4) : 0;
    const size_t need = 2 * words * 4 * (size_t) cap_alloc + cnt_bytes + req_bytes;
    if (int rc = workspace_reserve(h, need, s)) return rc;
    int32_t *cnt = reinterpret_cast<int32_t *>(h->d_ws);
    int32_t *req_cnt = cnt + (size_t) (kWfMaxDepth + 1) * kWfStageInts;
    PathStream st[2];
    for (int i = 0; i < 2; ++i) {
        float *b = reinterpret_cast<float *>(reinterpret_cast<char *>(h->d_ws) + cnt_bytes) + (size_t) i * words * cap_alloc;
        const long long c = cap_alloc;
        st[i].cap = c;
        st[i].pixel = reinterpret_cast<int32_t *>(b); st[i].slot = reinterpret_cast<uint32_t *>(b + c); st[i].tri = reinterpret_cast<int32_t *>(b + 2 * c);
        st[i].hu = b + 3 * c; st[i].hv = b + 4 * c; st[i].dir = b + 5 * c; st[i].beta = b + 8 * c; st[i].acc = b + (8 + 3 * (1 + K)) * c;
        st[i].hit = traced ? reinterpret_cast<float4 *>(b + (8 + 6 * (1 + K)) * c) : nullptr;
        st[i].prev_t = nullptr;
        st[i].binned = binned ? 1 : 0;
    }
    TraceQueue tq{};
    tq.req = traced ? reinterpret_cast<float4 *>(reinterpret_cast<char *>(h->d_ws) + cnt_bytes + 2 * words * 4 * (size_t) cap_alloc) : nullptr;
    if (!rec) h->slots[0] += (uint64_t) n;
    const float inv_spp = 1.f / (float) o->spp;
    const long long j_first = rec ? rec->c0 : 0;
    for (long long j0 = j_first; j0 < j_first + n; j0 += cap) {
        const long long cn = std::min(cap, j_first + n - j0);
        LaunchCtx cx;
        if (int rc = make_ctx(h, o, 0, cx)) return rc;
        HIP_TRY(hipMemsetAsync(cnt, 0, (size_t) (std::min(depth, kWfMaxDepth) + 1) * kWfStageInts * sizeof(int32_t), s));
        if (traced) HIP_TRY(hipMemsetAsync(req_cnt, 0, (size_t) (std::min(depth, kWfMaxDepth) + 1) * kWfSub * kWfCountStride * sizeof(int32_t), s));
        const int blocks = (launch_blocks(h, cn, wf_per_cu(cn)) + kWfSub - 1) / kWfSub * kWfSub;
        const long long trips = (cn + (long long) blocks * kBlock - 1) / ((long long) blocks * kBlock);
        st[0].sub_cap = st[1].sub_cap = binned ? binned_sub_cap : (blocks / kWfSub) * trips * kBlock;
        st[0].count = cnt;
        if constexpr ((FL & kSceneForest) != 0) {
            if (traced) {
                tq.sub_cap = 2 * st[0].sub_cap;
                tq.count = req_cnt;
                LaunchCtx cxp = cx;
                plan_lds(h, cxp, 1 << 30);
                cxp.sc.n_lnodes = cxp.sc.n_lbtris = cxp.sc.n_ltri = 0;
                const int dyn_p = cxp.off_stack;
                WfRec wr{};
                bool recording = false;
                if constexpr (K == 0) {
                    if (rec) { recording = true; wr = WfRec{rec->disk + (j0 - rec->c0), rec->stride, o->spp, o->spp_begin, nsp, j0, 0}; }
                }
                if (recording) {
                    if constexpr (K == 0)
                        hipLaunchKernelGGL(HIP_KERNEL_NAME(k_wf_camera<M, FL, true, true>), dim3(blocks), dim3(kBlock), lds_bytes(cx, h), s, cx, tv, o->spp, o->spp_begin, nsp, j0, cn,
                                           inv_spp, img, dimg, WH * 3, st[0], 1 | (depth == 1 ? 2 : 0), h->d_counters, make_rng_jump(o->rng_offset[0] + 2), tq, wr);
                } else
                hipLaunchKernelGGL(HIP_KERNEL_NAME(k_wf_camera<M, FL, true>), dim3(blocks), dim3(kBlock), lds_bytes(cx, h), s, cx, tv, o->spp, o->spp_begin, nsp, j0, cn,
                                   inv_spp, img, dimg, WH * 3, st[0], 1 | (depth == 1 ? 2 : 0), h->d_counters, make_rng_jump(o->rng_offset[0] + 2), tq, wr);
                HIP_TRY(hipGetLastError());
                for (int k = 0; k < depth; ++k) {
                    if (int rc = launch_wf_trace(h, tq.req, tq.count, tq.sub_cap, st[k & 1].hit, s)) return rc;
                    st[(k + 1) & 1].count = cnt + (size_t) (k + 1) * kWfStageInts;
                    tq.count = req_cnt + (size_t) (k + 1) * kWfSub * kWfCountStride;
                    cxp.jump = make_rng_jump(o->rng_offset[0] + 2 + 5 * (uint64_t) k);
                    wr.stage = k;
                    if (recording) {
                        if constexpr (K == 0)
                            hipLaunchKernelGGL(HIP_KERNEL_NAME(k_wf_bounce<M, FL, true, true>), dim3(blocks), dim3(kBlock), dyn_p, s, cxp, tv, inv_spp, img, dimg, WH * 3,
                                               st[k & 1], st[(k + 1) & 1], (k + 1 < depth ? 1 : 0) | (k + 2 == depth ? 2 : 0), h->d_counters, make_rng_jump(o->rng_offset[0] + 2 + 5 * (uint64_t) (k + 1)), tq, wr);
                    } else
                    hipLaunchKernelGGL(HIP_KERNEL_NAME(k_wf_bounce<M, FL, true>), dim3(blocks), dim3(kBlock), dyn_p, s, cxp, tv, inv_spp, img, dimg, WH * 3,
                                       st[k & 1], st[(k + 1) & 1], (k + 1 < depth ? 1 : 0) | (k + 2 == depth ? 2 : 0), h->d_counters, make_rng_jump(o->rng_offset[0] + 2 + 5 * (uint64_t) (k + 1)), tq, wr);
                    HIP_TRY(hipGetLastError());
                }
                continue;
            }
        }
        if (binned) {
            hipLaunchKernelGGL(HIP_KERNEL_NAME(k_wf_camera<M, FL>), dim3(blocks), dim3(kBlock), lds_bytes(cx, h), s, cx, tv, o->spp, o->spp_begin, nsp, j0, cn,
                               inv_spp, img, dimg, WH * 3, st[0], 1 | (depth == 1 ? 2 : 0), h->d_counters, make_rng_jump(o->rng_offset[0] + 2), tq, WfRec{});
            HIP_TRY(hipGetLastError());
            for (int k = 0; k < depth; ++k) {
                st[(k + 1) & 1].count = cnt + (size_t) (k + 1) * kWfStageInts;
                cx.jump = make_rng_jump(o->rng_offset[0] + 2 + 5 * (uint64_t) k);
                hipLaunchKernelGGL(HIP_KERNEL_NAME(k_wf_bounce<M, FL>), dim3(blocks), dim3(kBlock), lds_bytes(cx, h), s, cx, tv, inv_spp, img, dimg, WH * 3,
                                   st[k & 1], st[(k + 1) & 1], (k + 1 < depth ? 1 : 0) | (k + 2 == depth ? 2 : 0), h->d_counters, make_rng_jump(o->rng_offset[0] + 2 + 5 * (uint64_t) (k + 1)), tq, WfRec{});
                HIP_TRY(hipGetLastError());
            }
            continue;
        }
        hipLaunchKernelGGL(HIP_KERNEL_NAME(k_wf_camera<M, FL>), dim3(blocks), dim3(kBlock), lds_bytes(cx, h), s, cx, tv, o->spp, o->spp_begin, nsp, j0, cn,
                           inv_spp, img, dimg, WH * 3, st[0], (depth > 1 ? 1 : 0) | (depth == 2 ? 2 : 0), h->d_counters, make_rng_jump(o->rng_offset[0] + 2 + 5), tq, WfRec{});
        HIP_TRY(hipGetLastError());
        for (int k = 1; k < depth; ++k) {
            st[k & 1].count = cnt + (size_t) k * kWfStageInts;
            cx.jump = make_rng_jump(o->rng_offset[0] + 2 + 5 * (uint64_t) k);
            hipLaunchKernelGGL(HIP_KERNEL_NAME(k_wf_bounce<M, FL>), dim3(blocks), dim3(kBlock), lds_bytes(cx, h), s, cx, tv, inv_spp, img, dimg, WH * 3,
                               st[(k - 1) & 1], st[k & 1], (k + 1 < depth ? 1 : 0) | (k + 2 == depth ? 2 : 0), h->d_counters, make_rng_jump(o->rng_offset[0] + 2 + 5 * (uint64_t) (k + 1)), tq, WfRec{});
            HIP_TRY(hipGetLastError());
        }
    }
    return 0;
}

template <int K, int FL>
int run_camera_wavefront_geo(psdr_scene_s *h, const psdr_render_opts *o, const TangentView<K, FL> &tv, float *img, float *dimg, hipStream_t s) {
    const long long WH = (long long) h->desc.width * h->desc.height;
    const int nsp = o->spp_end - o->spp_begin;
    if (o->spp <= 0 || nsp <= 0) return 0;
    const long long n = WH * nsp;
    const int depth = o->max_depth;
    const size_t words = 8 + 6 * (1 + K) + 3 * K + 8;
    const long long cap = std::min(n, fit_chunk(launch_chunk(h, 26), 2 * words * 4 * 5 / 4 + 80, 64u << 20, h->ws_bytes));
// ... 357 lines not shown
```

psdr-cuda_amd/csrc/psdr_logd_lean.hip:

```cpp
#define PSDR_WIDE_TREE 0
#define PSDR_LEAF_PAIR 0
#include "psdr_kernels.h"
#include "psdr_logd_lean.h"

namespace {

constexpr int kLeanFlags = kSceneTiny;

template <int K, int FL, bool SEEDED>
__global__ __launch_bounds__(kBlock, PSDR_LOGD_WAVES_K1) void k_camera_logd_lean(LaunchCtx cx, TV<Dual<K>, FL> tv, int spp, int s_begin, SlotDiv nsp, long long n, float inv_spp,
                                                                                  float *__restrict__ img, float *__restrict__ dimg, long long plane, unsigned long long *counters, int own,
                                                                                  const ulonglong2 *__restrict__ seed) {
    constexpr int NV = 3 * (1 + K);
    if (counters[kLogdGateWord] != 1ull) return;
    TraversalStack st; setup_lds(cx, st, tv);
    Park pk{nullptr};
#if defined(__HIP_DEVICE_COMPILE__)
    pk.base = reinterpret_cast<float *>(psdr_dyn_lds + cx.off_park) + threadIdx.x;
#endif
    uint32_t nrays = 0;
    const long long nceil = (n + kBlock - 1) / kBlock * kBlock;
    for (long long jb = (long long) blockIdx.x * kBlock; jb < nceil; jb += (long long) gridDim.x * kBlock) {
        const long long j = jb + threadIdx.x;
        const bool in = j < n;
        int pixel = 0x7fffffff, s_in = 0;
        if (in) slot_to_pixel(j, nsp, pixel, s_in);
        Rng rng;
        if constexpr (SEEDED) {
            const ulonglong2 sd = in ? seed[j] : ulonglong2{0ull, 0ull};
            rng.init_seeded(sd.x, sd.y, cx.jump);
        } else {
            rng.init((uint64_t) pixel * (uint64_t) spp + (uint64_t) (s_begin + s_in), cx.jump);
        }
        const float j0 = rng.next(), j1 = rng.next();
        const int W = cx.sc.d.width;
        const float sx = ((float) (pixel % W) + j0) / (float) W, sy = ((float) (pixel / W) + j1) / (float) cx.sc.d.height;
        const TangentView<0, FL> tv0{};
        const RayT<float> ray = primary_ray<float>(cx.sc, tv0, sx, sy);
        const Vec3<Dual<K>> r = zero_nonfinite(li_path_logd_lean<K>(cx.sc, tv, st, cx.lp, rng, ray, in, nrays, pk));
        float v[NV];
        v[0] = in ? r.x.v * inv_spp : 0.f; v[1] = in ? r.y.v * inv_spp : 0.f; v[2] = in ? r.z.v * inv_spp : 0.f;
#pragma unroll
        for (int k = 0; k < K; ++k) { v[3 + 3 * k] = in ? r.x.d[k] * inv_spp : 0.f; v[4 + 3 * k] = in ? r.y.d[k] * inv_spp : 0.f; v[5 + 3 * k] = in ? r.z.d[k] * inv_spp : 0.f; }
        const bool head = wave_segmented_sum<NV>(pixel, v);
        if (head && in) {
            float *p = img + (size_t) pixel * 3;
            if (own) {
                p[0] = v[0]; p[1] = v[1]; p[2] = v[2];
#pragma unroll
                for (int k = 0; k < K; ++k) { float *q = dimg + (size_t) k * plane + (size_t) pixel * 3; q[0] = v[3 + 3 * k]; q[1] = v[4 + 3 * k]; q[2] = v[5 + 3 * k]; }
            } else {
                if (v[0] != 0.f) atomicAdd(p, v[0]);
                if (v[1] != 0.f) atomicAdd(p + 1, v[1]);
                if (v[2] != 0.f) atomicAdd(p + 2, v[2]);
#pragma unroll
                for (int k = 0; k < K; ++k) {
                    float *q = dimg + (size_t) k * plane + (size_t) pixel * 3;
                    if (v[3 + 3 * k] != 0.f) atomicAdd(q, v[3 + 3 * k]);
                    if (v[4 + 3 * k] != 0.f) atomicAdd(q + 1, v[4 + 3 * k]);
                    if (v[5 + 3 * k] != 0.f) atomicAdd(q + 2, v[5 + 3 * k]);
                }
            }
        }
    }
    count_rays(counters, nrays);
}

}

namespace psdr_host {
int logd_lean_launch_8(psdr_scene_s *h, const psdr_render_opts *o, const LaunchCtx &cx0, const psdr::TangentView<1, psdr::kSceneTiny> &tv, float *img, float *dimg, hipStream_t s, bool *ran) {
    *ran = false;
    if (h->opt.logd_park == 0) return 0;
    constexpr int kCuLds = 160 * 1024, park = ParkLayout<1>::cols * kBlock * 4;
    const int lds = (lds_bytes(cx0, h) + 15) / 16 * 16;
    const int limit = h->opt.lds_budget > 0 ? std::min(h->opt.lds_budget, kCuLds / PSDR_LOGD_WAVES_K1) : kCuLds / PSDR_LOGD_WAVES_K1;
    if (lds + park > limit) return 0;
    LaunchCtx cx = cx0;
    cx.off_park = lds;
    const long long WH = (long long) h->desc.width * h->desc.height;
    const int nsp = o->spp_end - o->spp_begin;
    const long long n = WH * nsp;
    const int own = wave_owns_pixels(h, nsp, n);
    const dim3 grid(launch_blocks(h, n, camera_blocks_per_cu(h, n)));
    const ulonglong2 *seed = seed_table(h, o, WH, nsp, n, s);
    if (seed != nullptr)
        hipLaunchKernelGGL(HIP_KERNEL_NAME(k_camera_logd_lean<1, kLeanFlags, true>), grid, dim3(kBlock), lds + park, s, cx, tv, o->spp, o->spp_begin, SlotDiv(nsp), n, 1.f / (float) o->spp, img, dimg,
                           WH * 3, h->d_counters, own, seed);
    else
        hipLaunchKernelGGL(HIP_KERNEL_NAME(k_camera_logd_lean<1, kLeanFlags, false>), grid, dim3(kBlock), lds + park, s, cx, tv, o->spp, o->spp_begin, SlotDiv(nsp), n, 1.f / (float) o->spp, img, dimg,
                           WH * 3, h->d_counters, own, seed);
    h->logd_lean_launches++;
    if (seed != nullptr) { h->logd_lean_seeded++; h->seed_launches++; }
    h->logd_lean_lds = lds; h->logd_lean_park = park;
    *ran = true;
    return 0;
}
}
```

psdr-cuda_amd/csrc/psdr_plan.h:

```cpp
#pragma once

namespace psdr_host {
inline int launch_blocks(const psdr_scene_s *h, long long n, int per_cu = 16) {
    const int forced = h->opt.blocks_per_cu;
    const long long need = (n + kBlock - 1) / kBlock;
    const long long cap = (long long) h->num_cus * (forced ? forced : per_cu);
    return (int) std::max(1LL, std::min(need, cap));
}

constexpr int kLdsBudget = 40 * 1024;
inline bool tiny_only(const psdr_scene_s *h) { return h->n_tiny > 0 && h->n_blas == 0; }
inline int emitter_faces(const psdr_scene_s *h) {
    int n = 0;
    for (int e = 0; e < h->desc.num_emitters && (size_t) (e + 1) * PSDR_EMITTER_I_STRIDE <= h->emitter_i.size(); ++e)
        n = std::max(n, h->emitter_i[(size_t) e * PSDR_EMITTER_I_STRIDE + 3] + h->emitter_i[(size_t) e * PSDR_EMITTER_I_STRIDE + 2]);
    return n;
}
constexpr int kLdsTexels = 256, kLdsTexelTangents = 3;
inline bool small_tables_fit(const psdr_scene_s *h) {
    const psdr_scene_desc &d = h->desc;
    return d.env_emitter < 0 && d.num_meshes <= 64 && d.num_bsdfs <= 32 && d.num_emitters >= 0 && d.num_emitters <= 8 &&
           (d.num_emitters == 0 || (d.face_cmf && d.face_pmf)) && emitter_faces(h) <= 64;
}
inline bool tiny_tables_ok(const psdr_scene_s *h) {
    return h->opt.tiny_variants != 0 && tiny_only(h) && small_tables_fit(h);
}
inline int scene_flag_set(const psdr_scene_s *h) {
    return (h->desc.env_emitter >= 0 ? kSceneEnv : 0) | (h->has_rough ? kSceneRough : 0) | (h->n_blas > 0 ? kSceneForest : 0) | (tiny_tables_ok(h) ? kSceneTiny : 0);
}
inline bool forest_tables(const psdr_scene_s *h) { return PSDR_FOREST_LDS_TABLES && h->n_blas > 0; }

inline int stack_entries_of(const psdr_scene_s *h) { return tiny_only(h) ? 0 : (h->wide ? h->stack_need4 + 1 : std::min(kBvhStack, h->bvh_depth + 2)); }
inline int staged_nodes_of(const psdr_scene_s *h) { return h->wide ? h->num_nodes4 : h->num_nodes; }
inline int plan_lds(const psdr_scene_s *h, LaunchCtx &cx, int reserved = 0) {
    const int forced = h->opt.lds_budget;
    const bool lean = !h->has_rough && h->desc.env_emitter < 0;
    const int budget = forced ? forced : (lean ? 28 * 1024 : kLdsBudget);
    const int stack_bytes = stack_entries_of(h) * kBlock * 4;
    int room = std::max(0, budget - reserved - stack_bytes);
    if (tiny_only(h)) room = std::max(room, staged_nodes_of(h) * kLdsNodeStride + h->num_btris * 48 + h->desc.num_tris * 96);
    SceneView &sc = cx.sc;
    int off = 0;
    sc.n_lnodes = std::min(staged_nodes_of(h), room / kLdsNodeStride); sc.off_lnodes = off; off += sc.n_lnodes * kLdsNodeStride; room -= sc.n_lnodes * kLdsNodeStride;
    sc.n_lbtris = (sc.n_lnodes == staged_nodes_of(h)) ? std::min(h->num_btris, room / 48) : 0;
    sc.off_lbtris = off; off += sc.n_lbtris * 48; room -= sc.n_lbtris * 48;
    sc.n_ltri = (sc.n_lbtris == h->num_btris) ? std::min(h->desc.num_tris, room / 96) : 0;
    sc.off_ltri = off; off += sc.n_ltri * 96;
    sc.off_lprim = off; off += h->n_tiny * kTinyHitWords * 4;
    sc.lt_trimesh = sc.lt_meshbsdf = sc.lt_meshemitter = sc.lt_bsdf = sc.lt_emf = sc.lt_emi = sc.lt_fcmf = sc.lt_fpmf = sc.lt_uv = sc.lt_tex = sc.lt_ecmf = sc.lt_epmf = -1;
    sc.lt_nfaces = 0; sc.lt_occ = -1; sc.occ = nullptr;
    const bool all_tables = tiny_tables_ok(h);
    if (all_tables || forest_tables(h)) {
        auto take = [&](int words) { const int o = off; off += (words * 4 + 15) / 16 * 16; return o; };
        const psdr_scene_desc &d = h->desc;
        sc.lt_nfaces = emitter_faces(h);
        if (all_tables) sc.lt_trimesh = take(d.num_tris);
        sc.lt_meshbsdf = take(d.num_meshes); sc.lt_meshemitter = take(d.num_meshes);
        sc.lt_bsdf = take(std::max(d.num_bsdfs, 1) * PSDR_BSDF_STRIDE);
        sc.lt_emf = take(d.num_emitters * PSDR_EMITTER_F_STRIDE); sc.lt_emi = take(d.num_emitters * PSDR_EMITTER_I_STRIDE);
        sc.lt_fcmf = take(sc.lt_nfaces); sc.lt_fpmf = take(sc.lt_nfaces);
        if (d.num_emitters > 1 && d.emitter_cmf && d.emitter_pmf) { sc.lt_ecmf = take(d.num_emitters); sc.lt_epmf = take(d.num_emitters); }
        if (all_tables && d.tri_uv) sc.lt_uv = take(d.num_tris * PSDR_TRIUV_STRIDE);
        if (d.num_texels > 0 && d.num_texels <= kLdsTexels) sc.lt_tex = take(d.num_texels * (1 + kLdsTexelTangents));
        if (all_tables && h->have_occ && h->d_occ != nullptr) { sc.occ = h->d_occ; sc.lt_occ = take(d.num_tris * d.num_tris); }
    }
    sc.lt_end = off;
    cx.off_stack = off;
    return off + stack_bytes;
}
inline int lds_bytes(const LaunchCtx &cx, const psdr_scene_s *h) { return cx.off_stack + stack_entries_of(h) * kBlock * 4; }
inline int plan_lds_no_walk(const psdr_scene_s *h, LaunchCtx &cx) {
    const int with_stacks = plan_lds(h, cx, 1 << 30);
    cx.sc.n_lnodes = cx.sc.n_lbtris = cx.sc.n_ltri = 0;
    return with_stacks;
}

inline bool open_scene(const psdr_scene_s *h) { return !(h->n_blas > 0 || (h->n_tiny > 0 && h->n_blas == 0)); }
inline bool traced_wavefront(const psdr_scene_s *h) { return h->traced_enabled && h->n_blas > 0 && h->num_nodes4 > 0 && h->d_nodes4 != nullptr; }
inline bool use_wavefront(const psdr_scene_s *h, const psdr_render_opts *o) {
    if (o->integrator != PSDR_INTEGRATOR_PATH || o->max_depth > 250) return false;
    if (h->desc.num_tris >= (1 << 29)) return false;
    if (o->flags & PSDR_FLAG_FUSED) return false;
    if (o->flags & PSDR_FLAG_WAVEFRONT) return true;
    if (o->max_depth < 2) return false;
    if (open_scene(h)) return true;
    const long long n = (long long) h->desc.width * h->desc.height * (o->spp_end - o->spp_begin);
    if (traced_wavefront(h)) return n >= (1ll << 16);
    return h->n_blas > 0 && h->wf_binned && n >= (1ll << 25);
}

inline SinkLayout make_sink_layout(const psdr_scene_s *h, const psdr_grads *g) {
    SinkLayout L{};
    int off = 0;
    L.cam_off = off; off += 16;
    if (g->g_env_f && h->desc.env_emitter >= 0) { L.env_off = off; L.env_n = PSDR_ENV_WORDS; off += PSDR_ENV_WORDS; }
    const int nt = h->desc.num_texels, nr = h->desc.num_emitters * 3;
    if (g->g_texels && nt > 0 && nt <= 2048) { L.tex_off = off; L.tex_n = nt; off += nt; }
    if (g->g_emitter_rad && nr > 0 && nr <= 256) { L.rad_off = off; L.rad_n = nr; off += nr; }
    if (g->g_tri_info && h->hot_rows > 0) {
        const int rows = std::min(h->hot_rows, (kSinkCacheWords - off) / PSDR_TRI_STRIDE);
        if (rows > 0) { L.hot_off = off; L.hot_rows = rows; L.hot_map = h->d_hot_map; L.hot_tris = h->d_hot_tris; off += rows * PSDR_TRI_STRIDE; }
    }
    L.total = off;
    L.stride = off | 1;
    L.rep = 1;
    const int max_rep = h->opt.sink_rep;
    while (L.rep * 2 <= max_rep && L.rep * 2 * L.stride <= kSinkCacheWords) L.rep *= 2;
    const bool priv_on = h->opt.sink_private != 0;
    L.priv_tri[0] = L.priv_tri[1] = -1; L.priv_slot[0] = L.priv_slot[1] = 0; L.priv_emitter = -1;
    if (priv_on && L.hot_rows > 0 && h->desc.num_emitters > 0 && h->desc.env_emitter != 0) {
        const int32_t *ei = h->emitter_i.data();
        const int n = std::min(std::min(ei[2], 2), L.hot_rows);
        for (int r = 0; r < n; ++r) { L.priv_tri[r] = ei[1] + r; L.priv_slot[r] = h->hot_identity ? ei[1] + r : r; }
        L.priv_rows = n;
        if (n > 0) { L.priv_off = (L.rep * L.stride + 3) / 4 * 4; if (L.rad_n) L.priv_emitter = 0; }
    }
    return L;
}

inline int camera_blocks_per_cu(const psdr_scene_s *h, long long n) {
    if (h->opt.camera_blocks > 0) return h->opt.camera_blocks;
    if (h->has_rough) return 16;
    if (h->n_tiny > 0 && h->n_blas == 0) return 40;
    const long long fit = n / ((long long) kBlock * h->num_cus * 2);
    return (int) std::max(16LL, std::min(64LL, fit));
}
inline int big_launch_per_cu(const psdr_scene_s *h, long long n) { return (int) std::max(16LL, std::min(40LL, n / ((long long) kBlock * h->num_cus * 8))); }
inline long long launch_chunk(const psdr_scene_s *h, int log2_default) { return 1ll << (h->opt.chunk_log2 > 0 ? h->opt.chunk_log2 : log2_default); }
inline bool probe_direct(const psdr_scene_s *h, const psdr_render_opts *o, long long n) {
    return traced_wavefront(h) && h->opt.probe != 0 && o->bsdf_samples == 1 && o->light_samples == 1 && !(o->flags & PSDR_FLAG_FUSED) && n >= (1ll << 16);
}
inline bool wave_owns_pixels(const psdr_scene_s *h, int nsp, long long chunk) {
    return h->opt.own_pixels != 0 && nsp <= 64 && 64 % nsp == 0 && chunk % nsp == 0;
}
inline bool path_sedge_split(const psdr_scene_s *h, long long n) {
    const int split_env = h->opt.sedge_split;
    return !(split_env == 0 || (split_env < 0 && n < (1ll << 18))) && n <= 0x7fffffffLL;
}
inline long long filter_grid_slots(long long n, int divisor) { return std::max(n / divisor, 1ll << 16); }
inline int primary_edge_replicas(long long pe_words, long long n) {
    int reps = 1;
    while (reps < 64 && (long long) (reps * 2) * pe_words * 4 <= (64ll << 20)) reps *= 2;
    return n < (1ll << 18) ? 1 : reps;
}

inline bool same_camera_samples(const psdr_render_opts &a, const psdr_render_opts &b) {
    return a.integrator == b.integrator && a.max_depth == b.max_depth && a.hide_emitters == b.hide_emitters && a.spp == b.spp && a.spp_begin == b.spp_begin &&
           a.spp_end == b.spp_end && a.rng_offset[0] == b.rng_offset[0] && ((a.flags ^ b.flags) & (PSDR_FLAG_FUSED | PSDR_FLAG_WAVEFRONT)) == 0;
}
inline int rev_record_words(int depth, bool wavefront) { return kRevDiskHead + (wavefront ? kRevDiskPerVertexCf : kRevDiskPerVertex) * depth; }
inline bool rev_launch_splits(const psdr_scene_s *h, const psdr_render_opts *o, long long n) {
    const int split_env = h->opt.rev_split;
    const bool replayable = o->integrator == PSDR_INTEGRATOR_PATH || (o->integrator == PSDR_INTEGRATOR_DIRECT && o->bsdf_samples <= 1 && o->light_samples <= 1);
    const bool has_tree = h->num_nodes > 0 && (h->n_tiny == 0 || h->n_blas > 0);
    const bool worth = o->integrator == PSDR_INTEGRATOR_PATH ? o->max_depth >= 2 : h->num_nodes >= 16384;
    return replayable && split_env != 0 && (split_env == 1 || (has_tree && worth && n >= (1ll << 20)));
}
inline bool rev_wavefront_sweep(const psdr_scene_s *h, const psdr_render_opts *o) {
    return o->integrator == PSDR_INTEGRATOR_PATH && std::min(o->max_depth, kMaxRevDepthDeep) <= kMaxRevDepth && traced_wavefront(h) && use_wavefront(h, o);
}
inline bool rev_value_sweep_is_wavefront(const psdr_scene_s *h, const psdr_render_opts *o, long long n) { return rev_launch_splits(h, o, n) && rev_wavefront_sweep(h, o); }

inline void rev_layout_of_sink(psdr_scene_s *h, const SinkLayout &L, bool deep_rec) {
    int32_t *r = h->rev_layout;
    r[0] = L.tex_n; r[1] = L.rad_n; r[2] = L.env_n; r[3] = L.hot_rows; r[4] = L.rep;
    r[5] = L.priv_rows; r[6] = L.priv_regs; r[7] = L.pend_rows;
    r[10] = h->hot_identity ? 1 : 0; r[11] = deep_rec ? 1 : 0; r[12] = L.priv_slot[0]; r[13] = L.priv_slot[1]; r[14] = h->hot_rows;
}

inline int plan_rev_one_vertex(const psdr_scene_s *h, LaunchCtx &cx, SinkLayout &L, int *dyn_bytes) {
    L.priv_rows = 0; L.priv_emitter = -1; L.priv_regs = 0;
    L.pend_rows = 0; L.pend_off = 0;
    const int cache_bytes = sink_bytes(L);
    plan_lds(h, cx, cache_bytes);
    cx.off_sink = lds_bytes(cx, h);
    *dyn_bytes = cx.off_sink + cache_bytes;
    if (*dyn_bytes > h->lds_limit) return fail("psdr_render_d_rev: the launch needs " + std::to_string(*dyn_bytes) + " bytes of LDS per workgroup (traversal stacks + gradient cache), the device offers " +
                                               std::to_string(h->lds_limit));
    return 0;
}

enum RevCameraForm { kRevFused = 0, kRevSplit = 1, kRevSplitWavefront = 2, kRevKeptRecords = 3, kRevProbe = 4 };
struct RevCameraPlan {
    int form, depth, rec_bytes, cache_bytes, dyn1, dyn_bytes;
    bool geo, deep_rec, split, kept_fused, no_tree;
};
inline int plan_rev_camera(psdr_scene_s *h, const psdr_render_opts *o, const psdr_grads *grads, long long n, int fl, bool reg_priv, bool value_only, bool has_out_img,
                           SinkLayout &L, LaunchCtx &cx, LaunchCtx &cx2, RevCameraPlan &p) {
    p.depth = o->integrator == PSDR_INTEGRATOR_PATH ? std::min(o->max_depth, kMaxRevDepthDeep) : 1;
    p.deep_rec = p.depth > kMaxRevDepth;
    p.rec_bytes = p.deep_rec ? 0 : p.depth * kPathRecWords * kBlock * 4;
    p.geo = value_only || grads->g_tri_info != nullptr || grads->g_cam_to_world != nullptr;
    const int wg_per_cu = (o->integrator == PSDR_INTEGRATOR_DIRECT && !(fl & kSceneRough)) ? 3 : 2;
    p.kept_fused = !value_only && p.geo && o->integrator == PSDR_INTEGRATOR_PATH && !p.deep_rec && h->opt.rev_split != 0 && h->kept.valid && h->kept.kind == 0 &&
                   h->kept.gen == h->tables_gen && h->kept.n == n && !has_out_img && same_camera_samples(h->kept.o, *o) && n <= launch_chunk(h, 26);
    p.split = value_only || p.kept_fused || (p.geo && rev_launch_splits(h, o, n));
    L.priv_regs = (p.geo && o->integrator == PSDR_INTEGRATOR_PATH && reg_priv) ? 1 : 0;
    cx2 = cx;
    const int stacks_only = plan_lds_no_walk(h, cx2);
    const int base2 = cx2.off_stack;
    const int floor_bytes = (p.split ? base2 : stacks_only) + p.rec_bytes;
    if (!L.priv_regs && L.priv_rows > 0 && floor_bytes + sink_bytes(L) > h->lds_limit / wg_per_cu) { L.priv_rows = 0; L.priv_emitter = -1; }
    L.pend_rows = 0; L.pend_off = 0;
    if (p.geo && h->opt.rev_sorted != 0 && grads->g_tri_info != nullptr && o->integrator == PSDR_INTEGRATOR_PATH) {
        for (int rows = std::min(p.depth, 4); rows >= 1; --rows) {
            SinkLayout t = L;
            sink_reserve_pending(t, rows);
            if (floor_bytes + sink_bytes(t) <= h->lds_limit / wg_per_cu) { L = t; break; }
        }
    }
    p.cache_bytes = sink_bytes(L);
    rev_layout_of_sink(h, L, p.deep_rec);
    plan_lds(h, cx, p.split ? p.rec_bytes : p.rec_bytes + p.cache_bytes);
    cx.off_pathrec = lds_bytes(cx, h);
    cx.off_sink = cx.off_pathrec + p.rec_bytes;
    cx2.off_pathrec = base2; cx2.off_sink = base2 + p.rec_bytes;
    p.no_tree = lds_bytes(cx, h) == cx.off_stack;
    if (p.split && p.no_tree) cx2 = cx;
    p.dyn1 = cx.off_pathrec + p.rec_bytes;
    p.dyn_bytes = (p.split ? cx2.off_sink : cx.off_sink) + p.cache_bytes;
    if (std::max(p.dyn_bytes, p.split ? p.dyn1 : 0) > h->lds_limit) return fail("psdr_render_d_rev: the launch needs " + std::to_string(p.dyn_bytes) + " bytes of LDS per workgroup (path record of " +
                                              std::to_string(p.depth) + " levels + traversal stacks + gradient cache), the device offers " + std::to_string(h->lds_limit));
    const bool forest = (fl & kSceneForest) != 0;
    const bool wf_value = forest && p.split && !value_only && !p.kept_fused && !p.no_tree && rev_wavefront_sweep(h, o);
    const bool direct_probe = forest && !p.split && !p.no_tree && o->integrator == PSDR_INTEGRATOR_DIRECT && probe_direct(h, o, n);
    p.form = p.split ? (wf_value ? kRevSplitWavefront : kRevSplit) : direct_probe ? kRevProbe : kRevFused;
    if (direct_probe) p.dyn_bytes = cx2.off_sink + p.cache_bytes;
    h->rev_layout[8] = p.form;
    return 0;
}
}
```

psdr-cuda_amd/psdr_cuda/_abi.py:

```python
import ctypes as C
import os

_HERE = os.path.dirname(os.path.abspath(__file__))
PKG_ROOT = os.path.dirname(_HERE)
REPO_ROOT = os.path.dirname(PKG_ROOT)

TRI_STRIDE = 24
TRIUV_STRIDE = 8
SEDGE_STRIDE = 16
PEDGE_STRIDE = 8
BSDF_STRIDE = 16
EMITTER_F_STRIDE = 8
EMITTER_I_STRIDE = 4
CAM_WORDS = 64
ENV_WORDS = 32
TRI_FACE_NORMALS = 0x40000000

BSDF_DIFFUSE, BSDF_ROUGHCONDUCTOR, BSDF_MICROFACET, BSDF_MICROFACET_NORMAL, BSDF_MICROFACET_HEIGHT = 0, 1, 2, 3, 4
SLOT_REFLECTANCE, SLOT_ALPHA_U, SLOT_ALPHA_V, SLOT_ETA, SLOT_K = range(5)
CAM_SAMPLE_TO_CAMERA, CAM_TO_WORLD, CAM_WORLD_TO_SAMPLE, CAM_POS, CAM_DIR, CAM_INV_AREA = 0, 16, 32, 48, 51, 54
INTEGRATOR_DIRECT, INTEGRATOR_PATH, INTEGRATOR_FIELD, INTEGRATOR_COLLOCATED, INTEGRATOR_POINT, INTEGRATOR_POINT_STACK = 0, 1, 2, 3, 4, 5
POINT_LIGHTS_MAX = 256
LIGHT_POINT, LIGHT_DISTANT = 0, 1
DISTANT_IN_ENV = "a distant light cannot reach a scene inside an environment map's bounding mesh (env_emitter >= 0)"
FLAG_FUSED, FLAG_WAVEFRONT, FLAG_LITERAL_FORMS, FLAG_KEEP_RECORDS, FLAG_PATH_SEDGES = 1, 2, 4, 8, 16
MAX_PATH_SEDGE_DEPTH = 8
FIELDS = {"silhouette": 0, "position": 1, "depth": 2, "geoNormal": 3, "shNormal": 4, "uv": 5}

_fp = C.c_void_p


class SceneDesc(C.Structure):
    _fields_ = [
        ("width", C.c_int32), ("height", C.c_int32),
        ("num_tris", C.c_int32), ("num_meshes", C.c_int32), ("num_bsdfs", C.c_int32), ("num_emitters", C.c_int32),
        ("num_sec_edges", C.c_int32), ("num_prim_edges", C.c_int32), ("num_texels", C.c_int32),
        ("num_guide_cells", C.c_int32),
        ("tri_info", _fp), ("tri_uv", _fp), ("tri_mesh", _fp), ("mesh_bsdf", _fp), ("mesh_emitter", _fp),
        ("bsdf_rec", _fp), ("texels", _fp), ("emitter_f", _fp), ("emitter_i", _fp),
        ("face_cmf", _fp), ("face_pmf", _fp), ("emitter_cmf", _fp), ("emitter_pmf", _fp),
        ("emitter_sum", C.c_float),
        ("cam", _fp),
        ("sec_edge", _fp), ("sec_cmf", _fp), ("sec_pmf", _fp), ("sec_sum", C.c_float),
        ("prim_edge", _fp), ("prim_cmf", _fp), ("prim_pmf", _fp), ("prim_sum", C.c_float),
        ("guide_reso", C.c_int32 * 3),
        ("guide_cmf", _fp), ("guide_pmf", _fp), ("guide_sum", C.c_float),
        ("env_emitter", C.c_int32), ("env_tex", C.c_int32 * 3), ("env_reso", C.c_int32 * 2),
        ("env_f", _fp), ("env_cmf", _fp), ("env_pmf", _fp), ("env_sum", C.c_float),
        ("material_mask", C.c_uint32),
        ("sec_edge_faces", _fp),
        ("prim_edge_z", _fp),
    ]


class RenderOpts(C.Structure):
    _fields_ = [
        ("integrator", C.c_int32), ("bsdf_samples", C.c_int32), ("light_samples", C.c_int32),
        ("max_depth", C.c_int32), ("hide_emitters", C.c_int32), ("field", C.c_int32),
        ("spp", C.c_int32), ("sppe", C.c_int32), ("sppse", C.c_int32),
        ("spp_begin", C.c_int32), ("spp_end", C.c_int32),
        ("sppe_begin", C.c_int32), ("sppe_end", C.c_int32),
        ("sppse_begin", C.c_int32), ("sppse_end", C.c_int32),
        ("flags", C.c_int32),
        ("rng_offset", C.c_uint64 * 3),
    ]


class Tangents(C.Structure):
    _fields_ = [("d_tri_info", _fp), ("d_texels", _fp), ("d_emitter_rad", _fp), ("d_cam_to_world", _fp),
                ("d_sec_edge", _fp), ("d_prim_edge", _fp), ("d_env_f", _fp)]


class Grads(C.Structure):
    _fields_ = [("g_tri_info", _fp), ("g_texels", _fp), ("g_emitter_rad", _fp), ("g_cam_to_world", _fp),
                ("g_sec_edge", _fp), ("g_prim_edge", _fp), ("g_env_f", _fp)]


class SmoothInfo(C.Structure):
    _fields_ = [("iterations", C.c_int32), ("converged", C.c_int32), ("form", C.c_int32), ("launches", C.c_int32), ("rel_residual", C.c_float * 3),
                ("one_workgroup_limit", C.c_int32), ("one_workgroup_default", C.c_int32), ("num_vertices", C.c_int32), ("num_entries", C.c_int32),
                ("long_rows", C.c_int32)]


SMOOTH_FORMS = {-1: "none", 0: "multi_launch", 1: "one_workgroup"}

TANGENT_FIELDS = ("tri_info", "texels", "emitter_rad", "cam_to_world", "sec_edge", "prim_edge", "env_f")

HIP_SYMBOLS = (
    "psdr_last_error", "psdr_version", "psdr_abi_struct_sizes", "psdr_scene_create", "psdr_scene_destroy", "psdr_scene_set_option", "psdr_scene_set_tables",
    "psdr_bvh_build", "psdr_bvh_stats", "psdr_scene_info", "psdr_trace", "psdr_render_c", "psdr_render_d_fwd", "psdr_render_d_rev",
    "psdr_guide_build", "psdr_scene_set_point_light", "psdr_scene_set_point_lights", "psdr_scene_set_light", "psdr_scene_set_lights", "psdr_scene_set_path_guide", "psdr_path_guide_build", "psdr_get_counters", "psdr_scene_rev_layout", "psdr_scene_seed_info", "psdr_scene_logd_info",
    "psdr_geo_world_vertices_fwd", "psdr_geo_world_vertices_rev", "psdr_geo_tri_rows_fwd", "psdr_geo_tri_rows_rev", "psdr_geo_sec_edges_fwd", "psdr_geo_sec_edges_rev", "psdr_geo_prim_edges_fwd", "psdr_geo_prim_edges_rev",
    "psdr_geo_compact_edges_fwd", "psdr_geo_compact_edges_rev", "psdr_geo_emitter_tables",
    "psdr_geo_world_vertices_jvp", "psdr_geo_tri_rows_jvp", "psdr_geo_sec_edges_jvp", "psdr_geo_prim_edges_jvp", "psdr_geo_compact_edges_jvp",
    "psdr_cube_sample_reuse", "psdr_sample_boundary_segment_direct",
    "psdr_smooth_create", "psdr_smooth_destroy", "psdr_smooth_set_option", "psdr_smooth_apply", "psdr_smooth_solve", "psdr_smooth_info",
)

HIP_LIB_PATH = os.path.join(PKG_ROOT, "lib", "libpsdr_hip.so")


def use_library(path):
    global HIP_LIB_PATH
    if _hip is not None:
        raise RuntimeError("psdr_cuda._abi.use_library: the library is already loaded (%s)" % HIP_LIB_PATH)
    HIP_LIB_PATH = os.path.abspath(path)


_hip = None


def load_hip():
    global _hip
    if _hip is not None:
        return _hip
    if not os.path.exists(HIP_LIB_PATH):
        raise RuntimeError("libpsdr_hip.so not built (%s): run `python -c 'import __graft_entry__ as g; g.build()'`"
                           % HIP_LIB_PATH)
    lib = C.CDLL(HIP_LIB_PATH)
    lib.psdr_last_error.restype = C.c_char_p
    lib.psdr_version.restype = C.c_char_p
    vp, i32 = C.c_void_p, C.c_int32
    lib.psdr_scene_create.argtypes = [C.POINTER(vp)]
    lib.psdr_scene_destroy.argtypes = [vp]
    lib.psdr_scene_set_option.argtypes = [vp, C.c_char_p, C.c_double]
    lib.psdr_scene_set_tables.argtypes = [vp, C.POINTER(SceneDesc)]
    lib.psdr_bvh_build.argtypes = [vp, vp]
    lib.psdr_trace.argtypes = [vp, i32] + [vp] * 7 + [vp] * 4 + [vp]
    lib.psdr_render_c.argtypes = [vp, C.POINTER(RenderOpts), vp, vp]
    lib.psdr_render_d_fwd.argtypes = [vp, C.POINTER(RenderOpts), i32, C.POINTER(Tangents), vp, vp, vp]
    lib.psdr_render_d_rev.argtypes = [vp, C.POINTER(RenderOpts), vp, vp, C.POINTER(Grads), vp]
    lib.psdr_guide_build.argtypes = [vp, C.POINTER(RenderOpts), C.POINTER(i32), i32, vp, vp]
    lib.psdr_scene_set_point_light.argtypes = [vp, C.POINTER(C.c_float), i32, C.POINTER(C.c_float), vp]
    lib.psdr_scene_set_point_lights.argtypes = [vp, i32, C.POINTER(C.c_float), i32, C.POINTER(C.c_float), vp]
    lib.psdr_scene_set_light.argtypes = [vp, i32, C.POINTER(C.c_float), i32, C.POINTER(C.c_float), vp]
    lib.psdr_scene_set_lights.argtypes = [vp, i32, C.POINTER(C.c_int32), C.POINTER(C.c_float), i32, C.POINTER(C.c_float), vp]
    lib.psdr_scene_set_path_guide.argtypes = [vp, C.POINTER(i32), vp, vp, C.c_float]
    lib.psdr_path_guide_build.argtypes = [vp, C.POINTER(RenderOpts), i32, C.POINTER(i32), i32, vp, vp]
    lib.psdr_get_counters.argtypes = [vp, C.POINTER(C.c_uint64)]
    lib.psdr_scene_info.argtypes = [vp, C.POINTER(i32)]
    lib.psdr_scene_rev_layout.argtypes = [vp, C.POINTER(i32)]
    lib.psdr_scene_seed_info.argtypes = [vp, C.POINTER(C.c_int64)]
    lib.psdr_scene_logd_info.argtypes = [vp, C.POINTER(C.c_int64)]
    lib.psdr_geo_world_vertices_fwd.argtypes = [i32, vp, vp, vp, vp, vp]
    lib.psdr_geo_world_vertices_rev.argtypes = [i32, vp, vp, vp, vp, vp, vp, vp]
    lib.psdr_geo_tri_rows_fwd.argtypes = [i32, i32, vp, vp, vp, vp, i32, vp]
    lib.psdr_geo_tri_rows_rev.argtypes = [i32, i32, vp, vp, vp, vp, i32, vp, vp, vp]
    lib.psdr_geo_sec_edges_fwd.argtypes = [i32, vp, vp, vp, i32, vp, vp, vp]
    lib.psdr_geo_sec_edges_rev.argtypes = [i32, vp, vp, vp, vp, i32, vp]
    lib.psdr_geo_prim_edges_fwd.argtypes = [i32, vp, vp, vp, vp, i32, vp, vp, vp, vp, vp]
    lib.psdr_geo_prim_edges_rev.argtypes = [i32, vp, vp, vp, vp, vp, vp, vp]
    lib.psdr_geo_compact_edges_fwd.argtypes = [i32, vp, i32, vp, i32, i32, vp, i32, i32, vp, vp, vp, vp, vp, vp, vp, vp]
    lib.psdr_geo_compact_edges_rev.argtypes = [i32, i32, vp, vp, vp, vp]
    lib.psdr_geo_world_vertices_jvp.argtypes = [i32, vp, vp, vp, vp, vp, vp, vp, vp]
    lib.psdr_geo_tri_rows_jvp.argtypes = [i32, i32, vp, vp, vp, vp, i32, vp, vp, vp]
    lib.psdr_geo_sec_edges_jvp.argtypes = [i32, vp, vp, vp, i32, vp, vp]
    lib.psdr_geo_prim_edges_jvp.argtypes = [i32, vp, vp, vp, vp, vp, vp, vp]
    lib.psdr_geo_compact_edges_jvp.argtypes = [i32, i32, vp, vp, vp, vp]
    lib.psdr_geo_emitter_tables.argtypes = [i32, vp, i32, vp, vp, i32, vp, vp, vp, vp, vp, vp, vp, vp, vp, vp]
    lib.psdr_cube_sample_reuse.argtypes = [i32, C.POINTER(i32), vp, vp, C.c_float, i32, i32, vp, vp, vp]
    lib.psdr_sample_boundary_segment_direct.argtypes = [C.POINTER(SceneDesc), i32] + [vp] * 12
    lib.psdr_smooth_create.argtypes = [i32, i32, vp, C.POINTER(vp)]
    lib.psdr_smooth_destroy.argtypes = [vp]
    lib.psdr_smooth_destroy.restype = None
    lib.psdr_smooth_set_option.argtypes = [vp, C.c_char_p, C.c_int]
    lib.psdr_smooth_apply.argtypes = [vp, C.c_float, vp, vp, vp]
    lib.psdr_smooth_solve.argtypes = [vp, C.c_float, vp, vp, vp, C.c_float, i32, vp]
    lib.psdr_smooth_info.argtypes = [vp, C.POINTER(SmoothInfo)]
    for name in HIP_SYMBOLS:
        if name not in ("psdr_last_error", "psdr_version", "psdr_smooth_destroy"):
            getattr(lib, name).restype = C.c_int
    sizes = (C.c_int32 * 4)()
    lib.psdr_abi_struct_sizes(sizes)
    mine = (C.sizeof(SceneDesc), C.sizeof(RenderOpts), C.sizeof(Tangents), C.sizeof(Grads))
    if tuple(sizes) != mine:
        raise RuntimeError("psdr_cuda/_abi.py is out of sync with include/psdr_hip.h: %s vs %s" % (tuple(sizes), mine))
    _hip = lib
    return lib


def check(lib, rc):
    if rc != 0:
        msg = lib.psdr_last_error()
        raise RuntimeError(msg.decode() if msg else "psdr_hip call failed (rc=%d)" % rc)


def scene_stats(handle):
    lib = load_hip()
    out = (C.c_int32 * 8)()
    check(lib, lib.psdr_scene_info(handle, out))
    return {"n_tiny": out[0], "n_blas": out[1], "n_inline": out[2], "leaf_tris": out[3], "device_built": out[4], "n_slab": out[5], "occ_rows": out[6], "occ_max_rows": out[7]}


REV_LAUNCH_KINDS = {-1: "none", 0: "fused", 1: "split", 2: "split_wavefront", 3: "kept_records", 4: "probe"}


def rev_layout(handle):
    lib = load_hip()
    out = (C.c_int32 * 16)()
    check(lib, lib.psdr_scene_rev_layout(handle, out))
    return {"tex_n": out[0], "rad_n": out[1], "env_n": out[2], "hot_rows": out[3], "rep": out[4], "priv_rows": out[5], "priv_regs": out[6],
            "pend_rows": out[7], "launch": REV_LAUNCH_KINDS[out[8]], "pe_reps": out[9], "hot_identity": out[10], "deep_rec": out[11],
            "priv_slot": (out[12], out[13]), "tree_hot_rows": out[14], "pe_sorted": out[15]}


def seed_cache_info(handle):
    lib = load_hip()
    out = (C.c_int64 * 4)()
    check(lib, lib.psdr_scene_seed_info(handle, out))
    return {"slots": int(out[0]), "bytes": int(out[1]), "fills": int(out[2]), "launches": int(out[3])}


def logd_info(handle):
    lib = load_hip()
    out = (C.c_int64 * 4)()
    check(lib, lib.psdr_scene_logd_info(handle, out))
    return {"launches": int(out[0]), "lean": int(out[1]), "lean_seeded": int(out[2]), "lean_lds_bytes": int(out[3])}


def make_opts(integrator=INTEGRATOR_DIRECT, bsdf_samples=1, light_samples=1, max_depth=1, hide_emitters=False,
              field=0, spp=1, sppe=0, sppse=0, spp_range=None, sppe_range=None, sppse_range=None,
              rng_offset=(0, 0, 0), flags=0):
    o = RenderOpts()
    o.flags = flags
    o.integrator, o.bsdf_samples, o.light_samples = integrator, bsdf_samples, light_samples
    o.max_depth, o.hide_emitters, o.field = max_depth, int(bool(hide_emitters)), field
    o.spp, o.sppe, o.sppse = spp, sppe, sppse
    o.spp_begin, o.spp_end = spp_range if spp_range is not None else (0, spp)
    o.sppe_begin, o.sppe_end = sppe_range if sppe_range is not None else (0, sppe)
    o.sppse_begin, o.sppse_end = sppse_range if sppse_range is not None else (0, sppse)
    for i in range(3):
        o.rng_offset[i] = int(rng_offset[i])
    return o


def draws_per_slot(opts):
    if opts.integrator == INTEGRATOR_DIRECT:
        li = 3 * opts.bsdf_samples + 2 * opts.light_samples
    elif opts.integrator == INTEGRATOR_PATH:
        li = 5 * opts.max_depth
    else:
        li = 0
    se = 3
    if opts.integrator == INTEGRATOR_PATH and (opts.flags & FLAG_PATH_SEDGES) and opts.max_depth >= 2:
        se = 11 * opts.max_depth - 9
    return (2 + li, 1 + 2 * li, se)
```

Measured before the change: 20750 Mpath-samples/s.

## Add lean path-tracer kernels for tiny slab-only diffuse scenes in renderC and logd

Adds specialized camera kernels (renderC twin and a logd K=1 twin) for scenes made only of axis-aligned tiny primitives with plain diffuse BSDFs. They intersect directly against kernarg-resident primitive rows, evaluate the albedo once per vertex, and park state in LDS only where needed, with a fixed launch bound of waves. The aim is to cut intersection overhead, register pressure and redundant texture/derivative evaluation. In exchange it adds a separate code path with gating conditions that fall back when the scene does not match, plus counters for tracking use.

```diff
diff --git a/__graft_entry__.py b/__graft_entry__.py
--- a/__graft_entry__.py
+++ b/__graft_entry__.py
@@ -38,6 +38,7 @@
     "lightstage": ("hostcheck/hostcheck_lightstage.cpp", "hostcheck/libhostcheck_lightstage.so", _product_and_harness, HOST_FLAGS),
     "distantlight": ("hostcheck/hostcheck_distantlight.cpp", "hostcheck/libhostcheck_distantlight.so", _product_and_harness, HOST_FLAGS),
     "plan": ("hostcheck/hostcheck_plan.cpp", "hostcheck/libhostcheck_plan.so", _product_and_harness, HOST_FLAGS),
+    "path_lean": ("hostcheck/hostcheck_path_lean.cpp", "hostcheck/libhostcheck_path_lean.so", _product_and_harness, HOST_FLAGS),
     "smooth": ("hostcheck/hostcheck_smooth.cpp", "hostcheck/libhostcheck_smooth.so", lambda: [os.path.join(CSRC, "psdr_smooth.h")], HOST_FLAGS),
     "poison": ("poison/poison.hip", "poison/libpoison.so", lambda: [], ["-O1"]),
 }
@@ -88,6 +89,10 @@
         o = os.path.join(obj_dir, "logd_lean.o")
         objs.append(o)
         unit_cmds[o] = ["hipcc"] + HIPCC_FLAGS + ["-c", os.path.join(csrc, "psdr_logd_lean.hip"), "-o", o]
+        jobs.append(subprocess.Popen(unit_cmds[o]))
+        o = os.path.join(obj_dir, "path_lean.o")
+        objs.append(o)
+        unit_cmds[o] = ["hipcc"] + HIPCC_FLAGS + ["-c", os.path.join(csrc, "psdr_path_lean.hip"), "-o", o]
         jobs.append(subprocess.Popen(unit_cmds[o]))
         o = os.path.join(obj_dir, "host.o")
         objs.append(o)
@@ -154,7 +159,7 @@
     srcs = [os.path.join(csrc, f) for f in os.listdir(csrc)] + [os.path.join(ROOT, "include", "psdr_hip.h")]
     obj_dir = os.path.join(PKG, "lib", "obj")
     defect_lib = os.path.join(ROOT, "tests", "poison", "libpsdr_hip_defect.so")
-    objs = [os.path.join(obj_dir, "%s%d.o" % (unit, v)) for v in VARIANTS for unit in ("variant", "path_sedge", "collocated", "pointlight", "lightstage")] + [os.path.join(obj_dir, "logd_lean.o"), os.path.join(obj_dir, "host.o"), os.path.join(obj_dir, "tables.o"), os.path.join(obj_dir, "smooth.o")]
+    objs = [os.path.join(obj_dir, "%s%d.o" % (unit, v)) for v in VARIANTS for unit in ("variant", "path_sedge", "collocated", "pointlight", "lightstage")] + [os.path.join(obj_dir, "logd_lean.o"), os.path.join(obj_dir, "path_lean.o"), os.path.join(obj_dir, "host.o"), os.path.join(obj_dir, "tables.o"), os.path.join(obj_dir, "smooth.o")]
     if not all(os.path.exists(o) for o in objs):
         return None
     if object_job is not None and object_job.wait() != 0:
diff --git a/include/psdr_hip.h b/include/psdr_hip.h
--- a/include/psdr_hip.h
+++ b/include/psdr_hip.h
@@ -246,6 +246,8 @@
 
 int psdr_scene_logd_info(psdr_scene_t h, int64_t out[4]);
 
+int psdr_scene_path_lean_info(psdr_scene_t h, int64_t out[4]);
+
 int psdr_get_counters(psdr_scene_t h, uint64_t out[4]);
 
 #ifdef __cplusplus
diff --git a/psdr-cuda_amd/csrc/psdr_hip.hip b/psdr-cuda_amd/csrc/psdr_hip.hip
--- a/psdr-cuda_amd/csrc/psdr_hip.hip
+++ b/psdr-cuda_amd/csrc/psdr_hip.hip
@@ -765,6 +765,7 @@
     else if (n == "logd") h->opt.logd = iv;
     else if (n == "seed_cache") h->opt.seed_cache = iv;
     else if (n == "logd_park") h->opt.logd_park = iv;
+    else if (n == "path_lean") h->opt.path_lean = iv;
     else if (n == "seed_cache_log2") h->opt.seed_cache_log2 = std::max(0, std::min(40, iv));
     else if (n == "keep_records") h->opt.keep_records = iv;
     else if (n == "rev_sorted") h->opt.rev_sorted = iv;
@@ -1299,6 +1300,11 @@
     out[0] = h->logd_launches; out[1] = h->logd_lean_launches; out[2] = h->logd_lean_seeded; out[3] = (int64_t) h->logd_lean_lds + h->logd_lean_park;
     return 0;
 }
+int psdr_scene_path_lean_info(psdr_scene_t h, int64_t out[4]) {
+    if (!h || !out) return fail("psdr_scene_path_lean_info: null argument");
+    out[0] = h->path_lean_launches[0]; out[1] = h->path_lean_launches[1]; out[2] = h->path_lean_fallbacks[0]; out[3] = h->path_lean_fallbacks[1];
+    return 0;
+}
 int psdr_scene_seed_info(psdr_scene_t h, int64_t out[4]) {
     if (!h || !out) return fail("psdr_scene_seed_info: null argument");
     out[0] = h->seed_valid ? h->seed_key[0] * h->seed_key[3] : 0; out[1] = (int64_t) (h->seed_cap * sizeof(ulonglong2)); out[2] = h->seed_fills; out[3] = h->seed_launches;
diff --git a/psdr-cuda_amd/csrc/psdr_host.h b/psdr-cuda_amd/csrc/psdr_host.h
--- a/psdr-cuda_amd/csrc/psdr_host.h
+++ b/psdr-cuda_amd/csrc/psdr_host.h
@@ -139,6 +139,7 @@
     int seed_cache = 1;
     int seed_cache_log2 = 25;
     int logd_park = 1;
+    int path_lean = 1;
     int bvh_maxleaf = 4;
     float bvh_tcost = 2.0f;
 };
@@ -230,6 +231,7 @@
     long long seed_fills = 0, seed_launches = 0;
     long long logd_launches = 0, logd_lean_launches = 0, logd_lean_seeded = 0;
     int logd_lean_lds = 0, logd_lean_park = 0;
+    long long path_lean_launches[2] = {0, 0}, path_lean_fallbacks[2] = {0, 0};
     void *d_ws = nullptr;
     size_t ws_bytes = 0;
     void *d_live = nullptr;
@@ -348,6 +350,7 @@
 const LightStageOps *light_stage_ops_8();
 const LightStageOps *light_stage_ops_10();
 int logd_lean_launch_8(psdr_scene_s *h, const psdr_render_opts *o, const LaunchCtx &cx, const psdr::TangentView<1, psdr::kSceneTiny> &tv, float *img, float *dimg, hipStream_t s, bool *ran);
+int path_lean_launch_8(psdr_scene_s *h, const psdr_render_opts *o, const LaunchCtx &cx, const psdr::TangentView<0, psdr::kSceneTiny> &tv, float *img, float *dimg, hipStream_t s, bool *ran);
 const VariantOps *variant_ops_0();
 const VariantOps *variant_ops_1();
 const VariantOps *variant_ops_2();
diff --git a/psdr-cuda_amd/csrc/psdr_kernels.h b/psdr-cuda_amd/csrc/psdr_kernels.h
--- a/psdr-cuda_amd/csrc/psdr_kernels.h
+++ b/psdr-cuda_amd/csrc/psdr_kernels.h
@@ -1629,6 +1629,13 @@
     hipLaunchKernelGGL(HIP_KERNEL_NAME(k_camera<G, R, INTEG, FL, NOTREE>), dim3(launch_blocks(h, n, camera_blocks_per_cu(h, n))), dim3(kBlock), lds_bytes(cx, h), s, cx, tv, o->spp, \
                        o->spp_begin, nsp, n, 1.f / (float) o->spp, img, dimg, WH * 3, h->d_counters, 0ll, ProbeView{nullptr, nullptr}, own)
 #define PSDR_LAUNCH_CAMERA(INTEG) PSDR_LAUNCH_CAMERA_T(INTEG, ((FL & kSceneTiny) != 0))
+    if constexpr (FL == kSceneTiny && seeded_render_c<G, R, FL>()) {
+        if (o->integrator == PSDR_INTEGRATOR_PATH) {
+            bool lean = false;
+            if (int rc = path_lean_launch_8(h, o, cx, tv, img, dimg, s, &lean)) return rc;
+            if (lean) { HIP_TRY(hipGetLastError()); return 0; }
+        }
+    }
     if constexpr (seeded_render_c<G, R, FL>()) {
         if (o->integrator == PSDR_INTEGRATOR_PATH) {
             if (const ulonglong2 *seed = seed_table(h, o, WH, nsp, n, s)) {
diff --git a/psdr-cuda_amd/csrc/psdr_logd_lean.hip b/psdr-cuda_amd/csrc/psdr_logd_lean.hip
--- a/psdr-cuda_amd/csrc/psdr_logd_lean.hip
+++ b/psdr-cuda_amd/csrc/psdr_logd_lean.hip
@@ -2,6 +2,7 @@
 #define PSDR_LEAF_PAIR 0
 #include "psdr_kernels.h"
 #include "psdr_logd_lean.h"
+#include "psdr_path_lean.h"
 
 namespace {
 
@@ -71,6 +72,8 @@
 namespace psdr_host {
 int logd_lean_launch_8(psdr_scene_s *h, const psdr_render_opts *o, const LaunchCtx &cx0, const psdr::TangentView<1, psdr::kSceneTiny> &tv, float *img, float *dimg, hipStream_t s, bool *ran) {
     *ran = false;
+    if (int rc = path_lean_launch<1>(h, o, cx0, tv, img, dimg, s, ran)) return rc;
+    if (*ran) return 0;
     if (h->opt.logd_park == 0) return 0;
     constexpr int kCuLds = 160 * 1024, park = ParkLayout<1>::cols * kBlock * 4;
     const int lds = (lds_bytes(cx0, h) + 15) / 16 * 16;
diff --git a/psdr-cuda_amd/csrc/psdr_path_lean.h b/psdr-cuda_amd/csrc/psdr_path_lean.h
--- /dev/null
+++ b/psdr-cuda_amd/csrc/psdr_path_lean.h
@@ -0,0 +1,346 @@
+#pragma once
+#include "psdr_logd_lean.h"
+
+#ifndef PSDR_PATH_LEAN_AB
+#define PSDR_PATH_LEAN_AB 0
+#endif
+
+namespace psdr {
+
+template <int K> struct LeanLayout {
+    static constexpr int result = 0, beta = 3, rd = 6, s = 6 + 3 * K, rng = 6 + 6 * K, vtx = 10 + 6 * K, rho = 13 + 6 * K, cols = 16 + 6 * K;
+};
+
+template <bool MASKED>
+__device__ __forceinline__ Hit lean_closest_hit(const SceneView &sc, const Vec3f &o, const Vec3f &d, uint32_t rows) {
+    Hit best; best.tri = -1; best.u = best.v = -1.f; best.t = INFINITY;
+    const Vec3f inv{1.f / d.x, 1.f / d.y, 1.f / d.z};
+    int best_i = kNoPrim;
+#if defined(__HIP_DEVICE_COMPILE__)
+    typedef __attribute__((address_space(4))) const float4 kernarg_float4;
+    const kernarg_float4 *prim_rows = (kernarg_float4 *) ((__attribute__((address_space(4))) const char *) __builtin_amdgcn_kernarg_segment_ptr() + offsetof(SceneView, tiny));
+    const int aa_cnt = sc.aa_cnt;
+    float4 ra[kAaSlots]; float hb[kAaSlots]; int pk[kAaSlots];
+#pragma unroll
+    for (int i = 0; i < kAaSlots; ++i) {
+        ra[i] = prim_rows[i * 4];
+        const float2 r = *(__attribute__((address_space(4))) const float2 *) &prim_rows[i * 4 + 1];
+        hb[i] = r.x; pk[i] = __float_as_int_hd(r.y);
+    }
+    const int cx = aa_cnt & 255, cy = (aa_cnt >> 8) & 255, cz = aa_cnt >> 16;
+#define PSDR_AA(AX, S) do { if (!MASKED || ((rows >> (S)) & 1u) != 0u) aa_prim_test<AX, false>(ra[S], hb[S], pk[S], 0, o, d, inv, best, best_i, -1, -1); } while (0)
+    if (cx > 0) { PSDR_AA(0, 0); if (cx > 1) { PSDR_AA(0, 1); if (cx > 2) PSDR_AA(0, 2); } }
+    if (cy > 0) { PSDR_AA(1, 3); if (cy > 1) { PSDR_AA(1, 4); if (cy > 2) PSDR_AA(1, 5); } }
+    if (cz > 0) { PSDR_AA(2, 6); if (cz > 1) { PSDR_AA(2, 7); if (cz > 2) PSDR_AA(2, 8); } }
+#undef PSDR_AA
+#else
+    (void) rows; (void) o; (void) inv;
+#endif
+    resolve_tiny_hit(sc, best, best_i);
+    return best;
+}
+template <bool MASKED, class TVT>
+__device__ __forceinline__ Its<float> lean_intersect(const SceneView &sc, const TVT &tv, TraversalStack &st, const RayT<float> &ray, bool active, uint32_t &nrays, int pre_slot, uint32_t rows = 0xffffffffu) {
+    if constexpr ((PSDR_PATH_LEAN_AB & 4) != 0) return intersect<float, TVT, MASKED>(sc, tv, st, ray, active, kDetached, nrays, -1, -1, pre_slot, rows);
+    Its<float> its;
+    its.valid = false; its.tri = its.mesh = -1; its.J = 1.f; its.t = INFINITY;
+    if (!active) return its;
+    nrays++;
+    Hit h;
+    if constexpr (MASKED) h = lean_closest_hit<true>(sc, ray.o, ray.d, wave_or_hd(rows));
+    else h = lean_closest_hit<false>(sc, ray.o, ray.d, rows);
+    if (h.tri < 0) return its;
+    fill_its_from_hit<float>(its, sc, tv, h, ray, kDetached);
+    return its;
+}
+__device__ __forceinline__ Vec3f lean_eval(const Vec3f &rho, const Its<float> &its, const Vec3f &wo) {
+    if (!(its.wi.z > 0.f && wo.z > 0.f)) return Vec3f(0.f);
+    return rho * (wo.z * kInvPi);
+}
+
+template <int K> struct LeanValue { float v[3 * (1 + K)]; };
+
+template <int K, bool PARKED, class TVT>
+__device__ __forceinline__ LeanValue<K> li_path_lean(const SceneView &sc, const TVT &tv, TraversalStack &st, const LiParams &lp, Rng &rng, const RayT<float> &ray, uint32_t &nrays, const Park &pk) {
+    using L = LeanLayout<K>;
+    using TV0 = TangentView<0, TVT::flags>;
+    static_assert(TVT::tiny && !TVT::has_env && !TVT::has_rough && TVT::k == K, "the twins serve the plain diffuse flag set of scenes without a tree");
+    constexpr int KA = K > 0 ? K : 1;
+    const TV0 tv0{};
+    auto fence = [] { if constexpr (PARKED) Park::fence(); };
+    constexpr bool ONCE = (PSDR_PATH_LEAN_AB & 1) == 0;
+    Its<float> its = lean_intersect<false>(sc, tv0, st, ray, true, nrays, kPrePrimaryRay);
+    bool active = its.valid;
+    Vec3f result = lp.hide_emitters ? Vec3f(0.f) : Le<float>(sc, tv0, its, active);
+    float rd[KA][3], s[KA][3];
+#pragma unroll
+    for (int k = 0; k < KA; ++k) { rd[k][0] = rd[k][1] = rd[k][2] = 0.f; s[k][0] = s[k][1] = s[k][2] = 0.f; }
+    Vec3f beta(1.f);
+    for (int depth = 0; depth < lp.max_depth; ++depth) {
+        int bsdf_id = active ? Tab<TVT::flags>::mesh_bsdf(sc, its.mesh) : 0;
+        bool act = active;
+        if (bsdf_id < 0) { act = false; bsdf_id = 0; }
+        const Bsdf<float, float> bsdf(sc, tv0, bsdf_id);
+        Vec3f rho(0.f);
+        if constexpr (!ONCE && K > 0) {
+            if (active) {
+                float g[KA][3];
+                albedo_logd<KA>(sc, tv, its, g);
+#pragma unroll
+                for (int k = 0; k < K; ++k) { s[k][0] += g[k][0]; s[k][1] += g[k][1]; s[k][2] += g[k][2]; }
+            }
+        }
+        if (ONCE && act) {
+            if constexpr (K == 0) rho = bsdf.tex3(sc, tv0, PSDR_SLOT_REFLECTANCE, its);
+            else {
+                const Bsdf<float, Dual<KA>> bsdf_d(sc, tv, bsdf_id);
+                const Vec3<Dual<KA>> r = bsdf_d.tex3(sc, tv, PSDR_SLOT_REFLECTANCE, its);
+                rho = Vec3f(r.x.v, r.y.v, r.z.v);
+                const float ix = r.x.v != 0.f ? 1.f / r.x.v : 0.f, iy = r.y.v != 0.f ? 1.f / r.y.v : 0.f, iz = r.z.v != 0.f ? 1.f / r.z.v : 0.f;
+#pragma unroll
+                for (int k = 0; k < K; ++k) { s[k][0] += r.x.d[k] * ix; s[k][1] += r.y.d[k] * iy; s[k][2] += r.z.d[k] * iz; }
+            }
+        }
+        const float sb0 = rng.next(), sb1 = rng.next(), sb2 = rng.next();
+        const float s0 = rng.next(), s1 = rng.next();
+        float sb1k = sb1, sb2k = sb2;
+        if constexpr (PARKED) {
+            pk.put3(L::result, result); pk.put3(L::beta, beta);
+#pragma unroll
+            for (int k = 0; k < K; ++k) {
+                pk.put(L::rd + 3 * k, rd[k][0]); pk.put(L::rd + 3 * k + 1, rd[k][1]); pk.put(L::rd + 3 * k + 2, rd[k][2]);
+                pk.put(L::s + 3 * k, s[k][0]); pk.put(L::s + 3 * k + 1, s[k][1]); pk.put(L::s + 3 * k + 2, s[k][2]);
+            }
+            pk.put64(L::rng, rng.state); pk.put64(L::rng + 2, rng.inc);
+            pk.put(L::vtx, sb1); pk.put(L::vtx + 1, sb2);
+            if constexpr (ONCE) pk.put3(L::rho, rho);
+        }
+        fence();
+        Vec3f c(0.f);
+        if (act) {
+            const PosSample<float> ps = sample_emitter_position<float>(sc, tv0, its.p, s0, s1, false);
+            Vec3f wo = ps.p - its.p;
+            const float d2 = dot(wo, wo), dist = safe_sqrt(d2);
+            wo = wo / dist;
+            const RayT<float> ray1{its.p, wo};
+            const Vec3f wl = its.sh.to_local(wo);
+            const bool lit = PSDR_SKIP_UNLIT ? (wl.z > 0.f && its.wi.z > 0.f) : true;
+            auto trace_light = [&]() {
+                if constexpr (PSDR_OCC_ROWS) return lean_intersect<true>(sc, tv0, st, ray1, ps.valid && lit, nrays, kPreLightRay, occ_rows(sc, its.tri, ps.tri));
+                else return lean_intersect<false>(sc, tv0, st, ray1, ps.valid && lit, nrays, kPreLightRay);
+            };
+            const Its<float> its1 = trace_light();
+            if (its1.valid && its1.t > dist - kShadowEpsilon && emitter_of(sc, tv0, its1) >= 0) {
+                Vec3f rho_l = rho;
+                if constexpr (PARKED && ONCE) rho_l = pk.get3(L::rho);
+                const float Gv = abs_(dot(its1.n, -wo)) / d2;
+                const Vec3f bsdf_val = (ONCE ? lean_eval(rho_l, its, wl) : bsdf.eval(sc, tv0, its, wl, true)) * to_m<float>(Gv * ps.J / ps.pdf);
+                float pdf1 = bsdf.pdf(sc, tv0, its, wl, true);
+                pdf1 = pdf1 * Gv;
+                const float w = mis_weight(float(ps.pdf), pdf1);
+                c = c + Le<float>(sc, tv0, its1, true) * bsdf_val * w;
+            }
+        }
+        if constexpr (PARKED) {
+            Park::fence();
+            sb1k = pk.get(L::vtx); sb2k = pk.get(L::vtx + 1);
+            Park::fence();
+            pk.put3(L::vtx, c);
+            Park::fence();
+        }
+        const float sb[3] = {sb0, sb1k, sb2k};
+        Its<float> nits; Vec3f nf(0.f); bool nvalid = false;
+        Vec3f lb(0.f); float wb = 0.f; bool a1b = false;
+        if (act) {
+            Vec3f wo_s; float pdf_s;
+            bool a1 = bsdf.sample(sc, tv0, its, sb, true, wo_s, pdf_s);
+            Vec3f shn = its.sh.n;
+            asm volatile("" : "+v"(shn.x), "+v"(shn.y), "+v"(shn.z));
+            const Frame<float> fr(shn);
+            const Vec3f dir1 = fr.s * wo_s.x + fr.t * wo_s.y + shn * wo_s.z;
+            const RayT<float> ray1{its.p, dir1};
+            const Its<float> its1 = lean_intersect<false>(sc, tv0, st, ray1, a1, nrays, kPreBsdfRay);
+            const bool a_hit = a1 && its1.valid;
+            a1 = a_hit && emitter_of(sc, tv0, its1) >= 0;
+            Vec3f bsdf_val(0.f); float pdf0(0.f);
+            if (a_hit) {
+                Vec3f rho_b = rho;
+                if constexpr (PARKED && ONCE) rho_b = pk.get3(L::rho);
+                bsdf_val = ONCE ? lean_eval(rho_b, its, wo_s) : bsdf.eval(sc, tv0, its, wo_s, true);
+                const float Gv = abs_(dot(its1.n, -ray1.d)) / sqr(its1.t);
+                pdf0 = pdf_s * Gv;
+                bsdf_val = bsdf_val / pdf_s;
+            }
+            if (a1) {
+                wb = mis_weight(pdf0, float(emitter_position_pdf(sc, tv0, its.p, its1)));
+                lb = Le<float>(sc, tv0, its1, true) * bsdf_val;
+            }
+            a1b = a1;
+            nits = its1; nf = bsdf_val; nvalid = a_hit;
+        }
+        if constexpr (PARKED) {
+            Park::fence();
+            c = pk.get3(L::vtx);
+            result = pk.get3(L::result); beta = pk.get3(L::beta);
+#pragma unroll
+            for (int k = 0; k < K; ++k) {
+                rd[k][0] = pk.get(L::rd + 3 * k); rd[k][1] = pk.get(L::rd + 3 * k + 1); rd[k][2] = pk.get(L::rd + 3 * k + 2);
+                s[k][0] = pk.get(L::s + 3 * k); s[k][1] = pk.get(L::s + 3 * k + 1); s[k][2] = pk.get(L::s + 3 * k + 2);
+            }
+            rng.state = pk.get64(L::rng); rng.inc = pk.get64(L::rng + 2);
+            Park::fence();
+        }
+        if (a1b) c = c + lb * wb;
+        if (active) {
+            if constexpr (K == 0) result = result + beta * c;
+            else {
+                const Vec3f bc = beta * c;
+                result = result + bc;
+#pragma unroll
+                for (int k = 0; k < K; ++k) {
+                    rd[k][0] = fmaf(bc.x, s[k][0], rd[k][0]); rd[k][1] = fmaf(bc.y, s[k][1], rd[k][1]); rd[k][2] = fmaf(bc.z, s[k][2], rd[k][2]);
+                }
+            }
+            active = nvalid;
+            if (active) {
+                beta = beta * nf;
+                if (!(beta.x != 0.f || beta.y != 0.f || beta.z != 0.f)) active = false;
+            }
+        }
+        its = nits;
+    }
+    LeanValue<K> out;
+    const bool fx = isfinite(result.x), fy = isfinite(result.y), fz = isfinite(result.z);
+    out.v[0] = fx ? result.x : 0.f; out.v[1] = fy ? result.y : 0.f; out.v[2] = fz ? result.z : 0.f;
+#pragma unroll
+    for (int k = 0; k < K; ++k) {
+        out.v[3 + 3 * k] = (fx && isfinite(rd[k][0])) ? rd[k][0] : 0.f;
+        out.v[4 + 3 * k] = (fy && isfinite(rd[k][1])) ? rd[k][1] : 0.f;
+        out.v[5 + 3 * k] = (fz && isfinite(rd[k][2])) ? rd[k][2] : 0.f;
+    }
+    return out;
+}
+
+}
+
+namespace {
+
+template <int K> constexpr bool path_lean_parked() { return psdr_host::path_lean_cols(K) > 0; }
+
+template <int K, bool SEEDED>
+__device__ __forceinline__ void camera_path_lean(const LaunchCtx &cx, const TangentView<K, kSceneTiny> &tv, int spp, int s_begin, const SlotDiv &wdiv, int n_pixels, float inv_spp,
+                                                 float *__restrict__ img, float *__restrict__ dimg, long long plane, unsigned long long *counters, const ulonglong2 *__restrict__ seed) {
+    constexpr int NV = 3 * (1 + K);
+    constexpr bool PARKED = path_lean_parked<K>();
+    if constexpr (K > 0) { if (counters[kLogdGateWord] != 1ull) return; }
+    TraversalStack st; setup_lds(cx, st, tv);
+    Park pk{nullptr};
+#if defined(__HIP_DEVICE_COMPILE__)
+    if constexpr (PARKED) pk.base = reinterpret_cast<float *>(psdr_dyn_lds + cx.off_park) + threadIdx.x;
+#endif
+    uint32_t nrays = 0;
+    const int lane = threadIdx.x & 63;
+    const int wave = __builtin_amdgcn_readfirstlane((int) (threadIdx.x >> 6));
+    constexpr int kWaves = kBlock / 64;
+    for (int pb = (int) blockIdx.x * kWaves; pb < n_pixels; pb += (int) gridDim.x * kWaves) {
+        const int pixel = pb + wave;
+        if (pixel >= n_pixels) continue;
+        Rng rng;
+        if constexpr (SEEDED) {
+            const ulonglong2 sd = (seed + (size_t) pixel * 64)[lane];
+            rng.init_seeded(sd.x, sd.y, cx.jump);
+        } else {
+            rng.init((uint64_t) pixel * (uint64_t) spp + (uint64_t) (s_begin + lane), cx.jump);
+        }
+        const float j0 = rng.next(), j1 = rng.next();
+        const TangentView<0, kSceneTiny> tv0{};
+        if constexpr ((PSDR_PATH_LEAN_AB & 2) != 0) {
+            int pl = pixel;
+            asm volatile("" : "+v"(pl));
+            const int W = cx.sc.d.width;
+            const float sx = ((float) (pl % W) + j0) / (float) W, sy = ((float) (pl / W) + j1) / (float) cx.sc.d.height;
+            const RayT<float> ray = primary_ray<float>(cx.sc, tv0, sx, sy);
+            const LeanValue<K> r = li_path_lean<K, PARKED>(cx.sc, tv, st, cx.lp, rng, ray, nrays, pk);
+            float v[NV];
+#pragma unroll
+            for (int i = 0; i < NV; ++i) v[i] = r.v[i] * inv_spp;
+            const bool head = wave_segmented_sum<NV>(pl, v);
+            if (head) {
+                float *p = img + (size_t) pl * 3;
+                if (cx.lp.max_depth >= 0) {
+                    p[0] = v[0]; p[1] = v[1]; p[2] = v[2];
+#pragma unroll
+                    for (int k = 0; k < K; ++k) { float *q = dimg + (size_t) k * plane + (size_t) pl * 3; q[0] = v[3 + 3 * k]; q[1] = v[4 + 3 * k]; q[2] = v[5 + 3 * k]; }
+                } else {
+#pragma unroll
+                    for (int i = 0; i < 3; ++i) if (v[i] != 0.f) atomicAdd(p + i, v[i]);
+#pragma unroll
+                    for (int k = 0; k < K; ++k)
+                        for (int i = 0; i < 3; ++i) if (v[3 + 3 * k + i] != 0.f) atomicAdd(dimg + (size_t) k * plane + (size_t) pl * 3 + i, v[3 + 3 * k + i]);
+                }
+            }
+            continue;
+        }
+        int py, px;
+        slot_to_pixel(pixel, wdiv, py, px);
+        const float sx = ((float) px + j0) / (float) cx.sc.d.width, sy = ((float) py + j1) / (float) cx.sc.d.height;
+        const RayT<float> ray = primary_ray<float>(cx.sc, tv0, sx, sy);
+        const LeanValue<K> r = li_path_lean<K, PARKED>(cx.sc, tv, st, cx.lp, rng, ray, nrays, pk);
+        float v[NV];
+#pragma unroll
+        for (int i = 0; i < NV; ++i) v[i] = wave_total(r.v[i] * inv_spp);
+        if (lane == 0) {
+            float *p = img + (size_t) pixel * 3;
+            p[0] = v[0]; p[1] = v[1]; p[2] = v[2];
+#pragma unroll
+            for (int k = 0; k < K; ++k) { float *q = dimg + (size_t) k * plane + (size_t) pixel * 3; q[0] = v[3 + 3 * k]; q[1] = v[4 + 3 * k]; q[2] = v[5 + 3 * k]; }
+        }
+    }
+    count_rays(counters, nrays);
+}
+template <bool SEEDED>
+__global__ __launch_bounds__(kBlock, kPathLeanWaves) void k_camera_path_lean(LaunchCtx cx, TangentView<0, kSceneTiny> tv, int spp, int s_begin, SlotDiv wdiv, int n_pixels, float inv_spp,
+                                                                              float *__restrict__ img, float *__restrict__ dimg, long long plane, unsigned long long *counters,
+                                                                              const ulonglong2 *__restrict__ seed) {
+    camera_path_lean<0, SEEDED>(cx, tv, spp, s_begin, wdiv, n_pixels, inv_spp, img, dimg, plane, counters, seed);
+}
+template <int K, bool SEEDED>
+__global__ __launch_bounds__(kBlock, kPathLeanWaves) void k_camera_logd_path_lean(LaunchCtx cx, TangentView<K, kSceneTiny> tv, int spp, int s_begin, SlotDiv wdiv, int n_pixels, float inv_spp,
+                                                                                   float *__restrict__ img, float *__restrict__ dimg, long long plane, unsigned long long *counters,
+                                                                                   const ulonglong2 *__restrict__ seed) {
+    static_assert(K >= 1, "the renderC twin is k_camera_path_lean");
+    camera_path_lean<K, SEEDED>(cx, tv, spp, s_begin, wdiv, n_pixels, inv_spp, img, dimg, plane, counters, seed);
+}
+
+}
+
+namespace psdr_host {
+template <int K>
+int path_lean_launch(psdr_scene_s *h, const psdr_render_opts *o, const LaunchCtx &cx0, const psdr::TangentView<K, psdr::kSceneTiny> &tv, float *img, float *dimg, hipStream_t s, bool *ran) {
+    *ran = false;
+    const long long WH = (long long) h->desc.width * h->desc.height;
+    const int nsp = o->spp_end - o->spp_begin;
+    const long long n = WH * nsp;
+    const int lds = (lds_bytes(cx0, h) + 15) / 16 * 16, park = path_lean_cols(K) * kBlock * 4;
+    if (path_lean_form(h, kSceneTiny, K, o->integrator, true, nsp, n, lds) != kPathLeanOwnSlab) { h->path_lean_fallbacks[K > 0]++; return 0; }
+    LaunchCtx cx = cx0;
+    cx.off_park = lds;
+    const dim3 grid(launch_blocks(h, n, camera_blocks_per_cu(h, n)));
+    const ulonglong2 *seed = seed_table(h, o, WH, nsp, n, s);
+    const SlotDiv wdiv(h->desc.width);
+    const float inv_spp = 1.f / (float) o->spp;
+#define PSDR_LAUNCH_LEAN(...) hipLaunchKernelGGL(HIP_KERNEL_NAME(__VA_ARGS__), grid, dim3(kBlock), lds + park, s, cx, tv, o->spp, o->spp_begin, wdiv, (int) WH, inv_spp, img, dimg, WH * 3, h->d_counters, seed)
+    if constexpr (K == 0) { if (seed != nullptr) PSDR_LAUNCH_LEAN(k_camera_path_lean<true>); else PSDR_LAUNCH_LEAN(k_camera_path_lean<false>); }
+    else { if (seed != nullptr) PSDR_LAUNCH_LEAN(k_camera_logd_path_lean<K, true>); else PSDR_LAUNCH_LEAN(k_camera_logd_path_lean<K, false>); }
+#undef PSDR_LAUNCH_LEAN
+    h->path_lean_launches[K > 0]++;
+    if (seed != nullptr) h->seed_launches++;
+    if (K > 0) {
+        h->logd_lean_launches++;
+        if (seed != nullptr) h->logd_lean_seeded++;
+        h->logd_lean_lds = lds; h->logd_lean_park = park;
+    }
+    *ran = true;
+    return 0;
+}
+}
diff --git a/psdr-cuda_amd/csrc/psdr_path_lean.hip b/psdr-cuda_amd/csrc/psdr_path_lean.hip
--- /dev/null
+++ b/psdr-cuda_amd/csrc/psdr_path_lean.hip
@@ -0,0 +1,10 @@
+#define PSDR_WIDE_TREE 0
+#define PSDR_LEAF_PAIR 0
+#include "psdr_kernels.h"
+#include "psdr_path_lean.h"
+
+namespace psdr_host {
+int path_lean_launch_8(psdr_scene_s *h, const psdr_render_opts *o, const LaunchCtx &cx, const psdr::TangentView<0, psdr::kSceneTiny> &tv, float *img, float *dimg, hipStream_t s, bool *ran) {
+    return path_lean_launch<0>(h, o, cx, tv, img, dimg, s, ran);
+}
+}
diff --git a/psdr-cuda_amd/csrc/psdr_plan.h b/psdr-cuda_amd/csrc/psdr_plan.h
--- a/psdr-cuda_amd/csrc/psdr_plan.h
+++ b/psdr-cuda_amd/csrc/psdr_plan.h
@@ -133,6 +133,35 @@
 inline bool wave_owns_pixels(const psdr_scene_s *h, int nsp, long long chunk) {
     return h->opt.own_pixels != 0 && nsp <= 64 && 64 % nsp == 0 && chunk % nsp == 0;
 }
+enum PathLeanForm { kPathLeanNone = 0, kPathLeanOwnSlab = 1 };
+#ifndef PSDR_PATH_LEAN_PARK_K0
+#define PSDR_PATH_LEAN_PARK_K0 0
+#endif
+constexpr int path_lean_cols(int K) { return (K == 0 && !PSDR_PATH_LEAN_PARK_K0) ? 0 : 16 + 6 * K; }
+constexpr int kPathLeanWaves = 6;
+struct PathLeanCase {
+    int flags, K, integrator, texels_only;
+    int nsp; long long chunk;
+    int n_tiny, aa_cnt, n_blas;
+    int lds_scene, lds_budget;
+    int own_pixels, path_lean, logd_park;
+};
+inline bool wave_is_pixel(int own_pixels, int nsp, long long chunk) { return own_pixels != 0 && nsp == 64 && chunk % nsp == 0; }
+inline bool slab_only(int n_tiny, int aa_cnt, int n_blas) { return n_blas == 0 && aa_cnt != 0 && n_tiny > 0 && n_tiny <= kAaSlots; }
+inline int path_lean_form(const PathLeanCase &c) {
+    if (c.path_lean == 0 || c.flags != kSceneTiny || c.integrator != PSDR_INTEGRATOR_PATH) return kPathLeanNone;
+    if (!(c.K == 0 || (c.K == 1 && c.texels_only != 0 && c.logd_park != 0))) return kPathLeanNone;
+    if (!wave_is_pixel(c.own_pixels, c.nsp, c.chunk) || !slab_only(c.n_tiny, c.aa_cnt, c.n_blas)) return kPathLeanNone;
+    constexpr int kCuLds = 160 * 1024;
+    const int limit = c.lds_budget > 0 ? std::min(c.lds_budget, kCuLds / kPathLeanWaves) : kCuLds / kPathLeanWaves;
+    const int park = path_lean_cols(c.K) * kBlock * 4;
+    if (park > 0 && c.lds_scene + park > limit) return kPathLeanNone;
+    return kPathLeanOwnSlab;
+}
+inline int path_lean_form(const psdr_scene_s *h, int flags, int K, int integrator, bool texels_only, int nsp, long long chunk, int lds_scene) {
+    const PathLeanCase c{flags, K, integrator, texels_only ? 1 : 0, nsp, chunk, h->n_tiny, h->aa_cnt, h->n_blas, lds_scene, h->opt.lds_budget, h->opt.own_pixels, h->opt.path_lean, h->opt.logd_park};
+    return path_lean_form(c);
+}
 inline bool path_sedge_split(const psdr_scene_s *h, long long n) {
     const int split_env = h->opt.sedge_split;
     return !(split_env == 0 || (split_env < 0 && n < (1ll << 18))) && n <= 0x7fffffffLL;
diff --git a/psdr-cuda_amd/psdr_cuda/_abi.py b/psdr-cuda_amd/psdr_cuda/_abi.py
--- a/psdr-cuda_amd/psdr_cuda/_abi.py
+++ b/psdr-cuda_amd/psdr_cuda/_abi.py
@@ -89,7 +89,7 @@
 HIP_SYMBOLS = (
     "psdr_last_error", "psdr_version", "psdr_abi_struct_sizes", "psdr_scene_create", "psdr_scene_destroy", "psdr_scene_set_option", "psdr_scene_set_tables",
     "psdr_bvh_build", "psdr_bvh_stats", "psdr_scene_info", "psdr_trace", "psdr_render_c", "psdr_render_d_fwd", "psdr_render_d_rev",
-    "psdr_guide_build", "psdr_scene_set_point_light", "psdr_scene_set_point_lights", "psdr_scene_set_light", "psdr_scene_set_lights", "psdr_scene_set_path_guide", "psdr_path_guide_build", "psdr_get_counters", "psdr_scene_rev_layout", "psdr_scene_seed_info", "psdr_scene_logd_info",
+    "psdr_guide_build", "psdr_scene_set_point_light", "psdr_scene_set_point_lights", "psdr_scene_set_light", "psdr_scene_set_lights", "psdr_scene_set_path_guide", "psdr_path_guide_build", "psdr_get_counters", "psdr_scene_rev_layout", "psdr_scene_seed_info", "psdr_scene_logd_info", "psdr_scene_path_lean_info",
     "psdr_geo_world_vertices_fwd", "psdr_geo_world_vertices_rev", "psdr_geo_tri_rows_fwd", "psdr_geo_tri_rows_rev", "psdr_geo_sec_edges_fwd", "psdr_geo_sec_edges_rev", "psdr_geo_prim_edges_fwd", "psdr_geo_prim_edges_rev",
     "psdr_geo_compact_edges_fwd", "psdr_geo_compact_edges_rev", "psdr_geo_emitter_tables",
     "psdr_geo_world_vertices_jvp", "psdr_geo_tri_rows_jvp", "psdr_geo_sec_edges_jvp", "psdr_geo_prim_edges_jvp", "psdr_geo_compact_edges_jvp",
@@ -142,6 +142,7 @@
     lib.psdr_scene_rev_layout.argtypes = [vp, C.POINTER(i32)]
     lib.psdr_scene_seed_info.argtypes = [vp, C.POINTER(C.c_int64)]
     lib.psdr_scene_logd_info.argtypes = [vp, C.POINTER(C.c_int64)]
+    lib.psdr_scene_path_lean_info.argtypes = [vp, C.POINTER(C.c_int64)]
     lib.psdr_geo_world_vertices_fwd.argtypes = [i32, vp, vp, vp, vp, vp]
     lib.psdr_geo_world_vertices_rev.argtypes = [i32, vp, vp, vp, vp, vp, vp, vp]
     lib.psdr_geo_tri_rows_fwd.argtypes = [i32, i32, vp, vp, vp, vp, i32, vp]
@@ -218,6 +219,13 @@
     return {"launches": int(out[0]), "lean": int(out[1]), "lean_seeded": int(out[2]), "lean_lds_bytes": int(out[3])}
 
 
+def path_lean_info(handle):
+    lib = load_hip()
+    out = (C.c_int64 * 4)()
+    check(lib, lib.psdr_scene_path_lean_info(handle, out))
+    return {"render_c": int(out[0]), "logd": int(out[1]), "render_c_fallback": int(out[2]), "logd_fallback": int(out[3])}
+
+
 def make_opts(integrator=INTEGRATOR_DIRECT, bsdf_samples=1, light_samples=1, max_depth=1, hide_emitters=False,
               field=0, spp=1, sppe=0, sppse=0, spp_range=None, sppe_range=None, sppse_range=None,
               rng_offset=(0, 0, 0), flags=0):
```

New measurement: 22500 Mpath-samples/s (median of 6 runs). +8.5%, better.
